# winddori2002/DEX-TTS

Hardware: AMD Instinct MI355X
Metric: mel-frames/s at n_timesteps=50, 80-ch mel (sampler only); RTF (higher is better)
Workload: dtype bf16; 1 GPU; gedex_b1: gedex_lj B=1/GPU T=512 n_timesteps=50 (BASELINE.json configs[1]); global_batch=1, frames=512, hipgraph=False, parallelism=1 GPU

## Files before the change

### dex_tts_amd/csrc/conv_down.hip

```cpp
#include "kernels.h"
#include <cstdlib>
#include "lp_util.h"
#include "kernels_lp.h"

namespace dex {
namespace DEX_LP_NS {

typedef float f32x16 __attribute__((ext_vector_type(16)));
typedef unsigned short u16;

namespace {
constexpr int CD_C = 64, CD_MPX = 64, CD_PXB = 144;
constexpr int CD_PL = CD_MPX + 1, CD_ROWB = 2 * CD_PL * CD_PXB;
constexpr int CD_NIT = (2 * CD_MPX + 1) * 8, CD_NL = (CD_NIT + 255) / 256;
}

template <bool ALP> struct CdRow;
template <> struct CdRow<true> { uint4 a[CD_NL]; float m[CD_NL]; };
template <> struct CdRow<false> { uint4 a[CD_NL]; uint4 c[CD_NL]; float m[CD_NL]; };

template <bool ALP, bool CLP>
#ifdef DEX_LP_WSPLIT
#define CD_WAVES_ATTR
#else
#define CD_WAVES_ATTR __attribute__((amdgpu_waves_per_eu(ALP ? 2 : 1, ALP ? 2 : 1)))
#endif
__global__ __launch_bounds__(256) CD_WAVES_ATTR void conv_down_kernel(const ConvDownP p) {
    constexpr int SPB = CLP ? 144 : 272, STG = CD_MPX * SPB, OCH = CLP ? 8 : 16, NS = CD_MPX * OCH / 256;
    extern __shared__ __attribute__((aligned(16))) unsigned char smem_cd[];
    unsigned char* ring = smem_cd;
    unsigned char* stage = smem_cd + 3 * CD_ROWB;
    float* bs = reinterpret_cast<float*>(stage + STG);
    const int DUMMY = 3 * CD_ROWB + STG + CD_C * 4;
    const int tid = threadIdx.x, lane = tid & 63, wave = tid >> 6;
    const int i = lane & 31, hh = lane >> 5;
    const int ct = wave & 1, pt = wave >> 1;
    const int seg = blockIdx.x % p.nseg, chunk = blockIdx.x / p.nseg, b = blockIdx.y;
    const int ow0 = seg * CD_MPX, Ho = p.H / 2, Wo = p.W / 2;
    const int r0 = chunk * p.rows_per_wg, r1 = min(Ho, r0 + p.rows_per_wg);
    const bool full_strip = ow0 + CD_MPX <= Wo;
    const u16* Xb = reinterpret_cast<const u16*>(p.X) + (long)b * p.xb + p.x_coff;
    const float* Xf = reinterpret_cast<const float*>(p.X) + (long)b * p.xb + p.x_coff;
    const float* mrow = p.inmask + (long)b * p.mask_bstride;

    int coff[CD_NL], roff[CD_NL]; float cmask[CD_NL];
#pragma unroll
    for (int j = 0; j < CD_NL; ++j) {
        const int q = tid + 256 * j;
        const int pc = q >> 3, c8 = (q & 7) * 8;
        const int wi = 2 * ow0 - 1 + pc;
        const bool ok = q < CD_NIT && (unsigned)wi < (unsigned)p.W;
        const int wc = ok ? wi : 0;
        coff[j] = wc * p.ldx + c8;
        cmask[j] = ok ? mrow[wc * p.inmask_ws] : 0.f;
        roff[j] = q < CD_NIT ? ((pc & 1) * CD_PL + (pc >> 1)) * CD_PXB + c8 * 2 : -1;
    }
    using Row = CdRow<ALP>;
    auto row_load = [&](int row, Row& R) __attribute__((always_inline)) {
        const bool rok = (unsigned)row < (unsigned)p.H;
        const int rc = __builtin_amdgcn_readfirstlane(rok ? row : 0);
#pragma unroll
        for (int j = 0; j < CD_NL; ++j) {
            if constexpr (ALP) R.a[j] = *reinterpret_cast<const uint4*>(Xb + (long)rc * p.W * p.ldx + coff[j]);
            else { const float* xf = Xf + (long)rc * p.W * p.ldx + coff[j]; R.a[j] = *reinterpret_cast<const uint4*>(xf); R.c[j] = *reinterpret_cast<const uint4*>(xf + 4); }
            R.m[j] = rok ? cmask[j] : 0.f;
        }
    };
    auto row_store = [&](int row, const Row& R) __attribute__((always_inline)) {
        const int slot = __builtin_amdgcn_readfirstlane((row + 1) % 3) * CD_ROWB;
#pragma unroll
        for (int j = 0; j < CD_NL; ++j) {
            const float m = R.m[j];
            uint4 v;
            if constexpr (ALP) {
                v.x = pack2_lp(lp_lo(R.a[j].x) * m, lp_hi(R.a[j].x) * m); v.y = pack2_lp(lp_lo(R.a[j].y) * m, lp_hi(R.a[j].y) * m);
                v.z = pack2_lp(lp_lo(R.a[j].z) * m, lp_hi(R.a[j].z) * m); v.w = pack2_lp(lp_lo(R.a[j].w) * m, lp_hi(R.a[j].w) * m);
            } else {
                v.x = pack2_lp(__uint_as_float(R.a[j].x) * m, __uint_as_float(R.a[j].y) * m); v.y = pack2_lp(__uint_as_float(R.a[j].z) * m, __uint_as_float(R.a[j].w) * m);
                v.z = pack2_lp(__uint_as_float(R.c[j].x) * m, __uint_as_float(R.c[j].y) * m); v.w = pack2_lp(__uint_as_float(R.c[j].z) * m, __uint_as_float(R.c[j].w) * m);
            }
            *reinterpret_cast<uint4*>(smem_cd + (roff[j] >= 0 ? slot + roff[j] : DUMMY)) = v;
        }
    };

    Row Ra, Rb;
    row_load(2 * r0 - 1, Ra);
    row_load(2 * r0, Rb);
    uint4 wr[36];
    {
        const uint4* Wf = reinterpret_cast<const uint4*>(p.Wfrag) + (long)ct * 36 * 64 + lane;
#pragma unroll
        for (int ks = 0; ks < 36; ++ks) wr[ks] = Wf[ks * 64];
    }
#ifdef DEX_LP_WSPLIT
    uint4 wl[36];
    {
        const uint4* Wf = reinterpret_cast<const uint4*>(p.Wfrag) + 2L * 36 * 64 + (long)ct * 36 * 64 + lane;
#pragma unroll
        for (int ks = 0; ks < 36; ++ks) wl[ks] = Wf[ks * 64];
    }
#endif
    if (tid < CD_C) bs[tid] = p.bias[tid];
    row_store(2 * r0 - 1, Ra);
    row_store(2 * r0, Rb);
    row_load(2 * r0 + 1, Ra);
    row_store(2 * r0 + 1, Ra);
    row_load(r0 + 1 < r1 ? 2 * r0 + 2 : -1, Ra);
    row_load(r0 + 1 < r1 ? 2 * r0 + 3 : -1, Rb);
    lds_barrier();

    for (int oh = r0; oh < r1; ++oh) {
        f32x16 acc;
#pragma unroll
        for (int r = 0; r < 16; ++r) acc[r] = 0.f;
#pragma unroll
        for (int kh = 0; kh < 3; ++kh) {
            const unsigned char* rowp = ring + __builtin_amdgcn_readfirstlane((2 * oh + kh) % 3) * CD_ROWB;
#pragma unroll
            for (int kw = 0; kw < 3; ++kw) {
                const unsigned char* xr = rowp + ((kw & 1) * CD_PL + pt * 32 + i + (kw >> 1)) * CD_PXB + hh * 16;
#pragma unroll
                for (int ks = 0; ks < 4; ++ks) {
                    const lp8 xv = *reinterpret_cast<const lp8*>(xr + ks * 32);
                    acc = DEX_MFMA_LP(__builtin_bit_cast(lp8, wr[(kh * 3 + kw) * 4 + ks]), xv, acc, 0, 0, 0);
#ifdef DEX_LP_WSPLIT
                    acc = DEX_MFMA_LP(__builtin_bit_cast(lp8, wl[(kh * 3 + kw) * 4 + ks]), xv, acc, 0, 0, 0);
#endif
                }
            }
        }
        lds_barrier();
#pragma unroll
        for (int g = 0; g < 4; ++g) {
            unsigned char* d = stage + (pt * 32 + i) * SPB + (ct * 32 + 8 * g + 4 * hh) * (CLP ? 2 : 4);
            const float4 b4 = *reinterpret_cast<const float4*>(bs + ct * 32 + 8 * g + 4 * hh);
            const float v0 = acc[4 * g] + b4.x, v1 = acc[4 * g + 1] + b4.y, v2 = acc[4 * g + 2] + b4.z, v3 = acc[4 * g + 3] + b4.w;
            if constexpr (CLP) *reinterpret_cast<uint2*>(d) = make_uint2(pack2_lp(v0, v1), pack2_lp(v2, v3));
            else *reinterpret_cast<float4*>(d) = make_float4(v0, v1, v2, v3);
        }
        row_store(2 * oh + 2, Ra);
        row_store(2 * oh + 3, Rb);
        lds_barrier();
        row_load(oh + 2 < r1 ? 2 * oh + 4 : -1, Ra);
        row_load(oh + 2 < r1 ? 2 * oh + 5 : -1, Rb);
        __builtin_amdgcn_sched_barrier(0);
        {
            uint4 ov[NS];
#pragma unroll
            for (int j = 0; j < NS; ++j) { const int q = tid + 256 * j; ov[j] = *reinterpret_cast<const uint4*>(stage + (q / OCH) * SPB + (q % OCH) * 16); }
            const long rowbase = (((long)b * Ho + oh) * Wo) * p.ldy + p.y_coff;
#define CD_OUT(pred_) _Pragma("unroll") for (int j = 0; j < NS; ++j) { \
                const int q = tid + 256 * j, wo = ow0 + q / OCH, e = wo * p.ldy + (q % OCH) * (CLP ? 8 : 4); \
                if (pred_) { if constexpr (CLP) *reinterpret_cast<uint4*>(reinterpret_cast<u16*>(p.Y) + rowbase + e) = ov[j]; \
                             else *reinterpret_cast<uint4*>(reinterpret_cast<float*>(p.Y) + rowbase + e) = ov[j]; } }
            if (full_strip) { CD_OUT(true) } else { CD_OUT(wo < Wo) }
#undef CD_OUT
        }
    }
}

bool conv_down_supported(int C, int H, int W, int ldx, int ldy, int x_coff) {
#if defined(DEX_LP_WSPLIT) && !defined(DEX_WS_HAVE_DOWN)
    return false;
#endif
   
    return C == CD_C && (ldx % 8) == 0 && (ldy % 8) == 0 && (x_coff % 8) == 0 && (H % 2) == 0 && (W % 2) == 0 && H >= 2 && W >= 2;
}

void launch_conv_down(const ConvDownP& p0, hipStream_t st) {
    g_last_symbol = "conv_down_kernel";
    ConvDownP p = p0;
    const int Ho = p.H / 2, Wo = p.W / 2;
    p.nseg = (Wo + CD_MPX - 1) / CD_MPX;
    const int target = knob_or("DEX_CONV_DOWN_WGS", 512);
    int nchunk = (target + p.nseg * p.B - 1) / (p.nseg * p.B);
    if (nchunk < 1) nchunk = 1;
    if (nchunk > Ho) nchunk = Ho;
    p.rows_per_wg = (Ho + nchunk - 1) / nchunk;
    nchunk = (Ho + p.rows_per_wg - 1) / p.rows_per_wg;
    const int lds = 3 * CD_ROWB + CD_MPX * (p.c_lp ? 144 : 272) + CD_C * 4 + 16;
    static bool attr = false;
    if (!attr) {
        constexpr int LMAX = 3 * CD_ROWB + CD_MPX * 272 + CD_C * 4 + 16;
        hipFuncSetAttribute(reinterpret_cast<const void*>(&conv_down_kernel<true, true>), hipFuncAttributeMaxDynamicSharedMemorySize, LMAX);
        hipFuncSetAttribute(reinterpret_cast<const void*>(&conv_down_kernel<true, false>), hipFuncAttributeMaxDynamicSharedMemorySize, LMAX);
        hipFuncSetAttribute(reinterpret_cast<const void*>(&conv_down_kernel<false, true>), hipFuncAttributeMaxDynamicSharedMemorySize, LMAX);
        hipFuncSetAttribute(reinterpret_cast<const void*>(&conv_down_kernel<false, false>), hipFuncAttributeMaxDynamicSharedMemorySize, LMAX);
        attr = true;
    }
    const dim3 grid(p.nseg * nchunk, p.B);
    if (p.a_lp) { if (p.c_lp) hipLaunchKernelGGL((conv_down_kernel<true, true>), grid, dim3(256), lds, st, p); else hipLaunchKernelGGL((conv_down_kernel<true, false>), grid, dim3(256), lds, st, p); }
    else { if (p.c_lp) hipLaunchKernelGGL((conv_down_kernel<false, true>), grid, dim3(256), lds, st, p); else hipLaunchKernelGGL((conv_down_kernel<false, false>), grid, dim3(256), lds, st, p); }
}

}
}
```

### dex_tts_amd/csrc/convt_up.hip

```cpp
#include "kernels.h"
#include <cstdlib>
#include "lp_util.h"
#include "kernels_lp.h"

namespace dex {
namespace DEX_LP_NS {

typedef float f32x16 __attribute__((ext_vector_type(16)));
typedef unsigned short u16;

namespace {

constexpr int CU_C = 64;
constexpr int CU_PXB = 144;

template <int MT, bool ALP, bool CLP>
struct CuGeom {
    static constexpr int MPX = 32 * MT, PC = MPX + 2, ROWB = PC * CU_PXB, RING = 4 * ROWB;
    static constexpr int OPX = 2 * MPX, SPB = CLP ? 144 : 272, STG = 2 * OPX * SPB;
    static constexpr int NL = (PC * 8 + 255) / 256;
    static constexpr int OCH = CLP ? 8 : 16;
    static constexpr int NS = 2 * OPX * OCH / 256;
    static constexpr int NB = NS < 8 ? NS : 8;
    static constexpr int LDS = RING + STG + 256;
};

template <int NL, int PC, bool ALP>
__device__ __forceinline__ void cu_row_load(const ConvTUpP& p, const void* Xb, const float* mrow, int row, int iw0, int tid,
                                            uint4 (&ra)[NL], uint4 (&rb)[ALP ? 1 : NL], float (&m)[NL]) {
    const bool rok = (unsigned)row < (unsigned)p.H;
    const int rc = rok ? row : 0;
#pragma unroll
    for (int j = 0; j < NL; ++j) {
        const int q = tid + 256 * j;
        const int px = q >> 3, c8 = (q & 7) * 8;
        const int iw = iw0 - 1 + px;
        const bool ok = rok && q < PC * 8 && (unsigned)iw < (unsigned)p.W;
        const int wc = ok ? iw : 0;
        const long e = ((long)rc * p.W + wc) * p.ldx + c8;
        if constexpr (ALP) ra[j] = *reinterpret_cast<const uint4*>(reinterpret_cast<const u16*>(Xb) + e);
        else {
            ra[j] = *reinterpret_cast<const uint4*>(reinterpret_cast<const float*>(Xb) + e);
            rb[j] = *reinterpret_cast<const uint4*>(reinterpret_cast<const float*>(Xb) + e + 4);
        }
        const float mv = mrow[wc * p.inmask_ws];
        m[j] = ok ? mv : 0.f;
    }
}
template <int NL, int PC, bool ALP>
__device__ __forceinline__ void cu_row_store(unsigned char* slot, int tid, const uint4 (&ra)[NL], const uint4 (&rb)[ALP ? 1 : NL], const float (&m)[NL]) {
#pragma unroll
    for (int j = 0; j < NL; ++j) {
        const int q = tid + 256 * j;
        const int px = q >> 3, c8 = (q & 7) * 8;
        uint4 v;
        if constexpr (ALP) {
            v.x = pack2_lp(lp_lo(ra[j].x) * m[j], lp_hi(ra[j].x) * m[j]); v.y = pack2_lp(lp_lo(ra[j].y) * m[j], lp_hi(ra[j].y) * m[j]);
            v.z = pack2_lp(lp_lo(ra[j].z) * m[j], lp_hi(ra[j].z) * m[j]); v.w = pack2_lp(lp_lo(ra[j].w) * m[j], lp_hi(ra[j].w) * m[j]);
        } else {
            v.x = pack2_lp(__uint_as_float(ra[j].x) * m[j], __uint_as_float(ra[j].y) * m[j]);
            v.y = pack2_lp(__uint_as_float(ra[j].z) * m[j], __uint_as_float(ra[j].w) * m[j]);
            v.z = pack2_lp(__uint_as_float(rb[j].x) * m[j], __uint_as_float(rb[j].y) * m[j]);
            v.w = pack2_lp(__uint_as_float(rb[j].z) * m[j], __uint_as_float(rb[j].w) * m[j]);
        }
        if (q < PC * 8) *reinterpret_cast<uint4*>(slot + px * CU_PXB + c8 * 2) = v;
    }
}

}

template <int MT, bool ALP, bool CLP>
__global__ __launch_bounds__(256) void convt_up_kernel(const ConvTUpP p) {
    using G = CuGeom<MT, ALP, CLP>;
    extern __shared__ __attribute__((aligned(16))) unsigned char smem_cu[];
    unsigned char* ring = smem_cu;
    unsigned char* stage = smem_cu + G::RING;
    float* bs = reinterpret_cast<float*>(smem_cu + G::RING + G::STG);
    const int tid = threadIdx.x, lane = tid & 63, wave = tid >> 6;
    const int i = lane & 31, hh = lane >> 5;
    const int ph = wave >> 1, pw = wave & 1;
    const int seg = blockIdx.x % p.nseg, chunk = blockIdx.x / p.nseg, b = blockIdx.y;
    const int iw0 = seg * G::MPX;
    const int r0 = chunk * p.rows_per_wg, r1 = min(p.H, r0 + p.rows_per_wg);
    const void* Xb = ALP ? static_cast<const void*>(reinterpret_cast<const u16*>(p.X) + (long)b * p.xb + p.x_coff)
                         : static_cast<const void*>(reinterpret_cast<const float*>(p.X) + (long)b * p.xb + p.x_coff);
    const float* mrow = p.inmask + (long)b * p.mask_bstride;
    const int OW = 2 * p.W;

    uint4 wr[2][16];
    {
        const uint4* Wf = reinterpret_cast<const uint4*>(p.Wfrag[wave]);
#pragma unroll
        for (int ct = 0; ct < 2; ++ct)
#pragma unroll
            for (int ks = 0; ks < 16; ++ks) wr[ct][ks] = Wf[(ct * 16 + ks) * 64 + lane];
    }
#ifdef DEX_LP_WSPLIT
    uint4 wl[2][16];
    {
        const uint4* Wf = reinterpret_cast<const uint4*>(p.Wfrag[wave]) + 2L * 16 * 64;
#pragma unroll
        for (int ct = 0; ct < 2; ++ct)
#pragma unroll
            for (int ks = 0; ks < 16; ++ks) wl[ct][ks] = Wf[(ct * 16 + ks) * 64 + lane];
    }
#endif
    uint4 ra[G::NL], rb[ALP ? 1 : G::NL];
    float rm[G::NL];
    {
        uint4 pa[3][G::NL], pb[3][ALP ? 1 : G::NL];
        float pm[3][G::NL];
#pragma unroll
        for (int d = 0; d < 3; ++d) cu_row_load<G::NL, G::PC, ALP>(p, Xb, mrow, r0 + d - 1, iw0, tid, pa[d], pb[d], pm[d]);
        const float bv = tid < CU_C ? p.bias[tid] : 0.f;
        cu_row_load<G::NL, G::PC, ALP>(p, Xb, mrow, r0 + 2 <= r1 ? r0 + 2 : -1, iw0, tid, ra, rb, rm);
#pragma unroll
        for (int d = 0; d < 3; ++d) cu_row_store<G::NL, G::PC, ALP>(ring + ((r0 + d) & 3) * G::ROWB, tid, pa[d], pb[d], pm[d]);
        if (tid < CU_C) bs[tid] = bv;
    }
    lds_barrier();

    for (int ih = r0; ih < r1; ++ih) {
        f32x16 acc[2][MT];
#pragma unroll
        for (int ct = 0; ct < 2; ++ct)
#pragma unroll
            for (int g = 0; g < 4; ++g) {
                const float4 b4 = *reinterpret_cast<const float4*>(bs + ct * 32 + 8 * g + 4 * hh);
#pragma unroll
                for (int pt = 0; pt < MT; ++pt) { acc[ct][pt][4 * g] = b4.x; acc[ct][pt][4 * g + 1] = b4.y; acc[ct][pt][4 * g + 2] = b4.z; acc[ct][pt][4 * g + 3] = b4.w; }
            }
#pragma unroll
        for (int ks = 0; ks < 16; ++ks) {
            const int tap = ks >> 2, th = tap >> 1, tw = tap & 1;
            const unsigned char* xr = ring + ((ih + ph - th + 1) & 3) * G::ROWB + (i + 1 + pw - tw) * CU_PXB + ((ks & 3) * 16 + hh * 8) * 2;
#pragma unroll
            for (int pt = 0; pt < MT; ++pt) {
                const lp8 xb = *reinterpret_cast<const lp8*>(xr + pt * 32 * CU_PXB);
#pragma unroll
                for (int ct = 0; ct < 2; ++ct) {
                    acc[ct][pt] = DEX_MFMA_LP(__builtin_bit_cast(lp8, wr[ct][ks]), xb, acc[ct][pt], 0, 0, 0);
#ifdef DEX_LP_WSPLIT
                    acc[ct][pt] = DEX_MFMA_LP(__builtin_bit_cast(lp8, wl[ct][ks]), xb, acc[ct][pt], 0, 0, 0);
#endif
                }
            }
        }
        lds_barrier();
#pragma unroll
        for (int ct = 0; ct < 2; ++ct)
#pragma unroll
            for (int pt = 0; pt < MT; ++pt)
#pragma unroll
                for (int g = 0; g < 4; ++g) {
                    unsigned char* d = stage + (ph * G::OPX + 2 * (pt * 32 + i) + pw) * G::SPB + (ct * 32 + 8 * g + 4 * hh) * (CLP ? 2 : 4);
                    if constexpr (CLP) *reinterpret_cast<uint2*>(d) = make_uint2(pack2_lp(acc[ct][pt][4 * g], acc[ct][pt][4 * g + 1]), pack2_lp(acc[ct][pt][4 * g + 2], acc[ct][pt][4 * g + 3]));
                    else *reinterpret_cast<float4*>(d) = make_float4(acc[ct][pt][4 * g], acc[ct][pt][4 * g + 1], acc[ct][pt][4 * g + 2], acc[ct][pt][4 * g + 3]);
                }
        cu_row_store<G::NL, G::PC, ALP>(ring + ((ih + 3) & 3) * G::ROWB, tid, ra, rb, rm);
        lds_barrier();
        cu_row_load<G::NL, G::PC, ALP>(p, Xb, mrow, ih + 3 <= r1 ? ih + 3 : -1, iw0, tid, ra, rb, rm);
        __builtin_amdgcn_sched_barrier(0);
#pragma unroll
        for (int h0 = 0; h0 < G::NS; h0 += G::NB) {
            uint4 ov[G::NB];
#pragma unroll
            for (int j = 0; j < G::NB; ++j) {
                const int q = tid + 256 * (h0 + j);
                const int row = q / (G::OPX * G::OCH), rem = q % (G::OPX * G::OCH);
                ov[j] = *reinterpret_cast<const uint4*>(stage + (row * G::OPX + rem / G::OCH) * G::SPB + (rem % G::OCH) * 16);
            }
#pragma unroll
            for (int j = 0; j < G::NB; ++j) {
                const int q = tid + 256 * (h0 + j);
                const int row = q / (G::OPX * G::OCH), rem = q % (G::OPX * G::OCH);
                const int ow = 2 * iw0 + rem / G::OCH;
                const long e = (((long)b * 2 * p.H + 2 * ih + row) * OW + ow) * p.ldy + p.y_coff + (rem % G::OCH) * (CLP ? 8 : 4);
                if (ow < OW) {
                    if constexpr (CLP) *reinterpret_cast<uint4*>(reinterpret_cast<u16*>(p.Y) + e) = ov[j];
                    else *reinterpret_cast<uint4*>(reinterpret_cast<float*>(p.Y) + e) = ov[j];
                }
            }
        }
    }
}

bool convt_up_supported(int C, int H, int W, int ldx, int ldy) {
#if defined(DEX_LP_WSPLIT) && !defined(DEX_WS_HAVE_UP)
    return false;
#endif
    return C == CU_C && (ldx % 8) == 0 && (ldy % 8) == 0 && H >= 1 && W >= 1; }

template <int MT, bool ALP, bool CLP>
static void cu_launch(ConvTUpP p, hipStream_t st) {
    using G = CuGeom<MT, ALP, CLP>;
    static_assert(G::NS % G::NB == 0, "output chunks");
    p.nseg = (p.W + G::MPX - 1) / G::MPX;
    const long tiles = (long)p.H * p.nseg * p.B;
    const int target = knob_or("DEX_CONVT_WGS", 512);
    int R = (int)((tiles + target - 1) / target);
    if (R < 1) R = 1;
    if (R > p.H) R = p.H;
    const int nchunk = (p.H + R - 1) / R;
    p.rows_per_wg = R;
    static bool attr = false;
    if (!attr) { hipFuncSetAttribute(reinterpret_cast<const void*>(&convt_up_kernel<MT, ALP, CLP>), hipFuncAttributeMaxDynamicSharedMemorySize, G::LDS); attr = true; }
    hipLaunchKernelGGL((convt_up_kernel<MT, ALP, CLP>), dim3(p.nseg * nchunk, p.B), dim3(256), G::LDS, st, p);
}

void launch_convt_up(const ConvTUpP& p, hipStream_t st) {
    g_last_symbol = "convt_up_kernel";
    const bool wide = knob_or("DEX_CONVT_MT", 0) == 2;
#define CU_GO(MT) do { if (p.a_lp && p.c_lp) cu_launch<MT, true, true>(p, st); else if (p.a_lp) cu_launch<MT, true, false>(p, st); \
                       else if (p.c_lp) cu_launch<MT, false, true>(p, st); else cu_launch<MT, false, false>(p, st); } while (0)
    if (wide) CU_GO(2); else CU_GO(1);
#undef CU_GO
}

}
}
```

### dex_tts_amd/csrc/dex_api.hip

```cpp
#include <hip/hip_runtime.h>
#include <cstdlib>

#include <cmath>
#include <cstdarg>
#include <atomic>
#include <cstdio>
#include <mutex>
#include <cstring>
#include <map>
#include <unordered_map>
#include <string_view>
#include <string>
#include <vector>

#include "../../include/dex_amd.h"
#include "kernels.h"
#include "weight_store.h"

using namespace dex;

namespace dex {
namespace {
const char* const KNOB_NAMES[] = {
    "DEX_CONV_STREAM", "DEX_CONV_PP", "DEX_CONV_SKIP_DEAD", "DEX_H_BF16", "DEX_ATTN_SEPARATE", "DEX_ATTN_Q64", "DEX_ATTN_Q64_TAIL", "DEX_ATTN_Q64_HALF", "DEX_DIT_XCDS", "DEX_ATTN_GENERIC", "DEX_RES2", "DEX_LP_INTER", "DEX_DIT_CHAIN",
    "DEX_DIT_CLUSTER", "DEX_DIT_CLUSTER_LOCAL", "DEX_ATTN_X_LP", "DEX_RES_X_LP", "DEX_CAT_LP", "DEX_XCD_MAP", "DEX_DEBUG_DROP_HANDOFF", "DEX_PATCH_FUSED",
    "DEX_CONV_DOWN", "DEX_CONVT_UP", "DEX_DEBUG_PLAN",
    "DEX_ATTN_SHARED_W8", "DEX_CONVT_MT", "DEX_CONVT_WGS", "DEX_CONV_DOWN_WGS", "DEX_CONV_REGW", "DEX_CONV_REGW_RES", "DEX_CONV_SMALL_MAX", "DEX_CONV_TH8",
    "DEX_CONV_W8", "DEX_DWCONV_CAP", "DEX_FINAL_CAP", "DEX_FIRST_CAP", "DEX_FIRST_MFMA", "DEX_GEMM_NWALK", "DEX_NWALK_SPLIT", "DEX_NWALK_BM", "DEX_POS_COL", "DEX_POS_COL_MIN",
    "DEX_POS_CT", "DEX_REGW_MIN_TILES", "DEX_REGW_WGS", "DEX_ROWCHAIN64", "DEX_ROWCHAIN64A", "DEX_TIV_CAP", "DEX_TV_CHAIN", "DEX_TIV_FOLD", "DEX_LINATTN_NSUB", "DEX_TV_FOLD", "DEX_OUT2_MIN", "DEX_NWALK_DMA",
    "DEX_LINATTN_HEADWAVES", "DEX_LINATTN_OUT2_HW", "DEX_CONV_ROUND1", "DEX_CONV_RESIDENT", "DEX_KVCTX_ROWS", "DEX_OUT2_ROWS", "DEX_PE_TOK", "DEX_NWALK_SMALL"};
constexpr int N_KNOBS = (int)(sizeof(KNOB_NAMES) / sizeof(KNOB_NAMES[0]));
int knob_parse(const char* e) {
    if (!e) return KNOB_UNSET;
    char* end = nullptr;
    const long v = strtol(e, &end, 10);
    if (end == e) {
        static bool warned = false;
        if (!warned) { warned = true; fprintf(stderr, "libdexamd: ignoring a DEX_* knob whose value '%s' is not an integer\n", e); }
        return KNOB_UNSET;
    }
    return (int)v;
}
struct KnobSnapshot {
    int v[N_KNOBS];
    KnobSnapshot() { for (int i = 0; i < N_KNOBS; ++i) v[i] = knob_parse(getenv(KNOB_NAMES[i])); }
};
thread_local const KnobSnapshot* t_knobs = nullptr;
struct WsplitScope {
    bool prev;
    explicit WsplitScope(bool on) : prev(g_lp_wsplit) { g_lp_wsplit = on; }
    ~WsplitScope() { g_lp_wsplit = prev; }
};
struct KnobScope {
    const KnobSnapshot* prev;
    explicit KnobScope(const KnobSnapshot* k) : prev(t_knobs) { t_knobs = k; }
    ~KnobScope() { t_knobs = prev; }
};
}
static int knob_index(const char* name) {
    static const std::unordered_map<std::string_view, int> idx = [] {
        std::unordered_map<std::string_view, int> m;
        for (int i = 0; i < N_KNOBS; ++i) m.emplace(KNOB_NAMES[i], i);
        return m;
    }();
    const auto it = idx.find(std::string_view(name));
    return it == idx.end() ? -1 : it->second;
}
int knob(const char* name) {
    if (t_knobs) {
        const int i = knob_index(name);
        if (i >= 0) return t_knobs->v[i];
    }
    return knob_parse(getenv(name));
}
}
static_assert(PREC_FP32 == DEX_PREC_FP32 && PREC_BF16 == DEX_PREC_BF16 && PREC_FP16 == DEX_PREC_FP16 && PREC_FP16X2 == DEX_PREC_FP16X2, "kernels.h mirrors DexPrecision");

namespace {
void xcd_map_probe();

struct TD { float* p; int ld; int coff; int C; int lp = 0; };

struct ResW { PackedW w1, w2, wr; const float *b1, *g1, *be1, *b2, *g2, *be2, *br, *mlp_w, *mlp_b; int cin, cout; };
constexpr int ATT_KSPLIT_MAX = 4;
static int att_split_cap(long tokens) { return tokens <= 20480 ? 8 : ATT_KSPLIT_MAX; }
static bool attention_q64_regime(int N, int B) {
    if (N < 1024) return dit_sep64_small_n(N, B) && dit_rowchain64_form(N, B, 0);
    const int ks = attention_q64_ksplit(N, B, att_split_cap((long)B * N));
    const int nt32 = (N + 31) / 32, ng = (nt32 + 7) / 8;
    return 2L * B * ng * ks >= 128;
}
struct LinW { PackedW wqkv; const float *wqkv_raw, *wout_raw, *bias_eff, *g; LpView wkv[3], wq_frag[3]; int C; };
struct DitBlockW { PackedW wqkv, wproj, wfc1, wfc2; const float *bqkv, *bproj, *bfc1, *bfc2, *ada_w, *ada_b; };

struct Prof { std::string name; hipEvent_t a, b; double flops, bytes; };
struct ProfAgg { std::string name; int calls; double ms, flops, bytes; };

struct Arena {
    char* base = nullptr; size_t off = 0, cap = 0; bool dry = true;
    void* take(size_t bytes) {
        off = (off + 255) & ~size_t(255);
        void* p = dry ? nullptr : (void*)(base + off);
        if (!dry && trace) fprintf(stderr, "plan[%d] off %zu bytes %zu\n", trace++, off, bytes);
        off += bytes;
        return p;
    }
    int trace = 0;
    float* f(size_t n) { return (float*)take(n * sizeof(float)); }
};

}

struct DexCtx : WeightStore {
    DexCtx() : WeightStore("") {}
    DexConfig cfg{};
    int lpi() const { return precision == DEX_PREC_FP16X2 ? 2 : precision == DEX_PREC_FP16 ? 1 : 0; }
    int lp_kind() const { return precision == DEX_PREC_BF16 ? 1 : 2; }
    bool lp() const { return precision != DEX_PREC_FP32; }
    bool tuned = true;
    int precision = DEX_PREC_FP32;
    std::vector<std::vector<ResW>> down_res, up_res;
    std::vector<LinW> down_lin, up_lin;
    std::vector<PackedW> down_ds_w;
    std::vector<std::vector<PackedW>> up_us_w;
    std::vector<const float*> down_ds_b, up_us_b;
    const float *fc_w3 = nullptr, *fc_w1 = nullptr;
    PackedW fin_w, pe_pw, fl_w, tv_wk, tv_wv, tv_wl;
    PackedW pos_w;
    const float *fin_b = nullptr, *fin_g = nullptr, *fin_be = nullptr, *fconv_w = nullptr, *fconv_b = nullptr;
    const float *pe_dw = nullptr, *pe_db = nullptr, *pe_pb = nullptr, *pos_b = nullptr, *freq_pos = nullptr;
    std::vector<DitBlockW> blocks;
    const float *fl_b = nullptr, *fl_ada_w = nullptr, *fl_ada_b = nullptr;
    const float *tv_wq_raw = nullptr;
    float *mel_basis = nullptr, *mel_filt = nullptr; void* mel_ws = nullptr; size_t mel_ws_bytes = 0;
    const int* last_xerr = nullptr;
    int* st_host = nullptr; hipEvent_t st_ev = nullptr; bool st_pending = false;
    struct Tap { std::string name; const float* p; std::vector<int64_t> shape; };
    std::vector<Tap> taps;
    bool prof_on = false;
    std::vector<Prof> prof;
    std::vector<ProfAgg> prof_agg;
    struct GraphEntry { std::vector<uint64_t> key; hipGraphExec_t exec; uint64_t stamp; const int* xerr; };
    std::vector<GraphEntry> graphs;
    uint64_t graph_clock = 0;
    void drop_graphs() { for (auto& g : graphs) hipGraphExecDestroy(g.exec); graphs.clear(); }
    template <typename F> int replay(const std::vector<uint64_t>& key, hipStream_t st, F&& enqueue);
    void reset_records() {
        taps.clear();
        if (prof_on) { for (auto& pr : prof) { hipEventDestroy(pr.a); hipEventDestroy(pr.b); } prof.clear(); prof_agg.clear(); }
    }
};

template <typename F> int DexCtx::replay(const std::vector<uint64_t>& key, hipStream_t st, F&& enqueue) {
    GraphEntry* hit = nullptr;
    for (auto& g : graphs) if (g.key == key) { hit = &g; break; }
    if (!hit) {
        constexpr size_t MAX_GRAPHS = 8;
        if (graphs.size() >= MAX_GRAPHS) {
            size_t lru = 0;
            for (size_t i = 1; i < graphs.size(); ++i) if (graphs[i].stamp < graphs[lru].stamp) lru = i;
            hipGraphExecDestroy(graphs[lru].exec);
            graphs.erase(graphs.begin() + lru);
        }
        hipGraph_t graph = nullptr;
        DEX_HIPCHK(this, hipStreamBeginCapture(st, hipStreamCaptureModeThreadLocal));
        const int rc = enqueue();
        hipError_t ec = hipStreamEndCapture(st, &graph);
        if (rc) { if (graph) hipGraphDestroy(graph); return rc; }
        if (ec != hipSuccess || !graph) return fail(DEX_ERR_HIP, "stream capture failed: %s", hipGetErrorString(ec));
        hipGraphExec_t exec = nullptr;
        ec = hipGraphInstantiate(&exec, graph, nullptr, nullptr, 0);
        hipGraphDestroy(graph);
        if (ec != hipSuccess) return fail(DEX_ERR_HIP, "hipGraphInstantiate failed: %s", hipGetErrorString(ec));
        graphs.push_back({key, exec, 0, last_xerr});
        hit = &graphs.back();
    }
    last_xerr = hit->xerr;
    hit->stamp = ++graph_clock;
    DEX_HIPCHK(this, hipGraphLaunch(hit->exec, st));
    DEX_HIPCHK(this, hipGetLastError());
    return DEX_OK;
}

namespace {

int stage_dim(const DexConfig& c, int i) { return c.dim * c.dim_mults[i]; }
int in_planes(const DexConfig& c) { return 2 + (c.n_spks > 1 ? 1 : 0); }
int mid_dim(const DexConfig& c) { return stage_dim(c, c.n_stages - 1); }
int mid_h(const DexConfig& c) { return c.n_feats >> (c.n_stages - 1); }
int grid_h(const DexConfig& c) { return mid_h(c) / c.dit_stride; }
int token_rows(const DexConfig& c) { return (mid_h(c) + 2 * (c.dit_patch / 2) - c.dit_patch) / c.dit_stride + 1; }
int token_cols(const DexConfig& c, int wmid) {
    const int p = c.dit_patch, s = c.dit_stride;
    const int wp = (wmid % p == 0) ? wmid : wmid + (p - wmid % p);
    return (wp + 2 * (p / 2) - p) / s + 1;
}
int mlp_hidden(const DexConfig& c) { return (int)(c.dit_hidden * c.dit_mlp_ratio); }

void add_resnet(DexCtx* x, const std::string& p, int cin, int cout, int tdim) {
    x->add(p + ".mlp.1.weight", {cout, tdim}); x->add(p + ".mlp.1.bias", {cout});
    for (int blk = 1; blk <= 2; ++blk) {
        const std::string q = p + ".block" + std::to_string(blk) + ".block";
        x->add(q + ".0.weight", {cout, blk == 1 ? cin : cout, 3, 3}); x->add(q + ".0.bias", {cout});
        x->add(q + ".1.weight", {cout}); x->add(q + ".1.bias", {cout});
    }
    if (cin != cout) { x->add(p + ".res_conv.weight", {cout, cin, 1, 1}); x->add(p + ".res_conv.bias", {cout}); }
}
void add_linattn(DexCtx* x, const std::string& p, int c) {
    x->add(p + ".fn.g", {1});
    x->add(p + ".fn.fn.to_qkv.weight", {384, c, 1, 1});
    x->add(p + ".fn.fn.to_out.weight", {c, 128, 1, 1});
    x->add(p + ".fn.fn.to_out.bias", {c});
}
void build_inventory(DexCtx* x) {
    const DexConfig& c = x->cfg;
    const int d = c.dim;
    x->add("mlp.0.weight", {4 * d, d}); x->add("mlp.0.bias", {4 * d});
    x->add("mlp.2.weight", {d, 4 * d}); x->add("mlp.2.bias", {d});
    if (c.variant == DEX_VARIANT_DEX)
        for (const char* n : {"mlp_adap", "mlp_adap_sty"}) {
            const std::string s(n);
            x->add(s + ".0.weight", {d, d}); x->add(s + ".0.bias", {d});
            x->add(s + ".2.weight", {2 * d, d}); x->add(s + ".2.bias", {2 * d});
        }
    if (c.n_spks > 1) {
        const int e = c.spk_emb_dim;
        x->add("spk_mlp.0.weight", {4 * e, e}); x->add("spk_mlp.0.bias", {4 * e});
        x->add("spk_mlp.2.weight", {c.n_feats, 4 * e}); x->add("spk_mlp.2.bias", {c.n_feats});
    }
    for (int i = 0; i < c.n_stages; ++i) {
        const int ci = i == 0 ? in_planes(c) : stage_dim(c, i - 1), co = stage_dim(c, i);
        const std::string p = "downs." + std::to_string(i);
        add_resnet(x, p + ".0", ci, co, d); add_resnet(x, p + ".1", co, co, d); add_linattn(x, p + ".2", co);
        if (i < c.n_stages - 1) { x->add(p + ".3.conv.weight", {co, co, 3, 3}); x->add(p + ".3.conv.bias", {co}); }
    }
    const int hid = c.dit_hidden, mid = mid_dim(c), mh = mlp_hidden(c);
    x->add("vit.freq_new_pos_embed", {1, hid, grid_h(c), 1});
    x->add("vit.x_embedder.proj.0.weight", {mid, 1, c.dit_patch, c.dit_patch}); x->add("vit.x_embedder.proj.0.bias", {mid});
    x->add("vit.x_embedder.proj.2.weight", {hid, mid, 1, 1}); x->add("vit.x_embedder.proj.2.bias", {hid});
    x->add("vit.t_embedder.mlp.0.weight", {hid, 256}); x->add("vit.t_embedder.mlp.0.bias", {hid});
    x->add("vit.t_embedder.mlp.2.weight", {hid, hid}); x->add("vit.t_embedder.mlp.2.bias", {hid});
    x->add("vit.pos_conv.0.weight", {hid, hid / c.dit_conv_pos_groups, c.dit_conv_pos, c.dit_conv_pos});
    x->add("vit.pos_conv.0.bias", {hid});
    for (int k = 0; k < c.dit_depth; ++k) {
        const std::string p = "vit.blocks." + std::to_string(k);
        x->add(p + ".attn.qkv.weight", {3 * hid, hid}); x->add(p + ".attn.qkv.bias", {3 * hid});
        x->add(p + ".attn.proj.weight", {hid, hid}); x->add(p + ".attn.proj.bias", {hid});
        x->add(p + ".mlp.fc1.weight", {mh, hid}); x->add(p + ".mlp.fc1.bias", {mh});
        x->add(p + ".mlp.fc2.weight", {hid, mh}); x->add(p + ".mlp.fc2.bias", {hid});
        x->add(p + ".adaLN_modulation.1.weight", {6 * hid, hid}); x->add(p + ".adaLN_modulation.1.bias", {6 * hid});
    }
    const int so = c.dit_stride * c.dit_stride * mid;
    x->add("vit.final_layer.linear.weight", {so, hid}); x->add("vit.final_layer.linear.bias", {so});
    x->add("vit.final_layer.adaLN_modulation.1.weight", {2 * hid, hid}); x->add("vit.final_layer.adaLN_modulation.1.bias", {2 * hid});
    if (c.variant == DEX_VARIANT_DEX) {
        for (const char* w : {"w_q", "w_k", "w_v", "linear"}) x->add(std::string("tv_adaptor.") + w + ".weight", {mid, mid});
        for (const char* s : {"mean_sap", "std_sap"}) {
            x->add(std::string("tiv_adaptor.") + s + ".W.weight", {1, mid});
            x->add(std::string("tiv_adaptor.") + s + ".W.bias", {1});
        }
    }
    for (int j = 0; j < c.n_stages - 1; ++j) {
        const int i = c.n_stages - 1 - j;
        const int ci = stage_dim(c, i - 1), co = stage_dim(c, i);
        const std::string p = "ups." + std::to_string(j);
        add_resnet(x, p + ".0", co * 2, ci, d); add_resnet(x, p + ".1", ci, ci, d); add_linattn(x, p + ".2", ci);
        x->add(p + ".3.conv.weight", {ci, ci, 4, 4}); x->add(p + ".3.conv.bias", {ci});
    }
    x->add("final_block.block.0.weight", {d, d, 3, 3}); x->add("final_block.block.0.bias", {d});
    x->add("final_block.block.1.weight", {d}); x->add("final_block.block.1.bias", {d});
    x->add("final_conv.weight", {1, d, 1, 1}); x->add("final_conv.bias", {1});
}

__global__ void pack_convt_kernel(const float* src, float* dst, int Cin, int Cout) {
    const long total = 4L * 4 * Cin * Cout;
    for (long i = (long)blockIdx.x * blockDim.x + threadIdx.x; i < total; i += (long)gridDim.x * blockDim.x) {
        const int co = (int)(i % Cout);
        const int ci = (int)((i / Cout) % Cin);
        const int tap = (int)((i / ((long)Cout * Cin)) % 4);
        const int par = (int)(i / ((long)Cout * Cin * 4));
        const int ph = par >> 1, pw = par & 1, th = tap >> 1, tw = tap & 1;
        const int kh = (ph ? 0 : 1) + 2 * th, kw = (pw ? 0 : 1) + 2 * tw;
        dst[i] = src[(((long)ci * Cout + co) * 4 + kh) * 4 + kw];
    }
}

}

extern "C" {

const char* dex_version(void) { return "dexamd 0.1 (gfx950)"; }

int dex_ctx_create(const DexConfig* cfg, DexCtx** out) {
    if (!cfg || !out) return DEX_ERR_ARG;
    DexCtx* x = new DexCtx();
    x->cfg = *cfg;
    const DexConfig& c = x->cfg;
    *out = x;
    if (c.n_feats != 80) return x->fail(DEX_ERR_ARG, "n_feats must be 80 (diffusion.py:226 hard-codes it)");
    if (c.n_stages < 2 || c.n_stages > 4) return x->fail(DEX_ERR_ARG, "n_stages must be in [2,4]");
    if (c.dim != 64 && c.dim != 128) return x->fail(DEX_ERR_ARG, "dim must be 64 (GeDEX, DEX-VCTK/ESD) or 128 (DEX-LibriTTS)");
    if (c.dit_heads < 1 || c.dit_hidden % c.dit_heads || !attention_head_dim_supported(c.dit_hidden / c.dit_heads))
        return x->fail(DEX_ERR_ARG, "DiT head_dim must be 64, 128, 192 or 256 (hidden %d heads %d)", c.dit_hidden, c.dit_heads);
    if (c.dit_hidden % 64 || c.dit_hidden > 512) return x->fail(DEX_ERR_ARG, "dit_hidden must be a multiple of 64, <= 512");
    if (mlp_hidden(c) % 64) return x->fail(DEX_ERR_ARG, "mlp hidden must be a multiple of 64");
    if (c.dit_conv_pos_groups < 1 || c.dit_hidden % c.dit_conv_pos_groups || (c.dit_hidden / c.dit_conv_pos_groups) % 16 ||
        c.dit_hidden / c.dit_conv_pos_groups > 64)
        return x->fail(DEX_ERR_ARG, "pos-conv groups must be 16, 32, 48 or 64 channels wide");
    if (c.dit_conv_pos % 2) return x->fail(DEX_ERR_ARG, "conv_pos must be even");
    if (c.variant == DEX_VARIANT_DEX && !attention_head_dim_supported(mid_dim(c)))
        return x->fail(DEX_ERR_ARG, "DEX adaptors need mid_dim 64, 128, 192 or 256 (the cross-attention's head_dim)");
    x->tuned = c.dim == 64 && c.dit_hidden == 256 && c.dit_heads == 2 && c.dit_hidden / c.dit_conv_pos_groups == 32 &&
               (c.variant != DEX_VARIANT_DEX || mid_dim(c) == 128);
    build_inventory(x);
    xcd_map_probe();
    return DEX_OK;
}

void dex_ctx_destroy(DexCtx* x) {
    if (!x) return;
    x->release();
    if (x->mel_basis) hipFree(x->mel_basis);
    if (x->mel_filt) hipFree(x->mel_filt);
    if (x->mel_ws) hipFree(x->mel_ws);
    x->drop_graphs();
    for (auto& pr : x->prof) { hipEventDestroy(pr.a); hipEventDestroy(pr.b); }
    if (x->st_ev) hipEventDestroy(x->st_ev);
    if (x->st_host) hipHostFree(x->st_host);
    delete x;
}

const char* dex_last_error(const DexCtx* x) { return x ? x->err.c_str() : "null context"; }
int dex_ctx_num_weights(const DexCtx* x) { return x ? (int)x->keys.size() : 0; }
// ... 1608 lines not shown
```

### dex_tts_amd/csrc/dit_elem.hip

```cpp
#include "kernels.h"
#include <cstdlib>

namespace dex {

__device__ __forceinline__ float silu_d(float x) { return x * __builtin_amdgcn_rcpf(1.f + __expf(-x)); }
__device__ __forceinline__ float gelu_d(float x) { return 0.5f * x * (1.0f + erff(x * 0.70710678118654752440f)); }

template <int KS>
__global__ __launch_bounds__(256) void dwconv_silu_kernel(const DwConvP p) {
    extern __shared__ __attribute__((aligned(16))) float4 wsh_dw[];
    const int C4 = p.C >> 2;
    for (int q = threadIdx.x; q < KS * KS * C4; q += 256) wsh_dw[q] = *reinterpret_cast<const float4*>(p.Wd + (long)q * 4);
    __syncthreads();
    const long total = (long)p.B * p.Hf * p.Wt * C4;
    for (long gid = (long)blockIdx.x * 256 + threadIdx.x; gid < total; gid += (long)gridDim.x * 256) {
        const int cq = (int)(gid % C4);
        const long tok = gid / C4;
        const int wt = (int)(tok % p.Wt);
        const int f = (int)((tok / p.Wt) % p.Hf);
        const int b = (int)(tok / ((long)p.Wt * p.Hf));
        const float* X = p.X + (long)b * p.xb;
        const float* mrow = p.mask ? p.mask + (long)b * p.mask_bstride : nullptr;
        float mkc[KS]; int wcl[KS];
#pragma unroll
        for (int kw = 0; kw < KS; ++kw) {
            const int wi = wt * p.s + kw - p.pad;
            const bool inw = (unsigned)wi < (unsigned)p.Wi;
            wcl[kw] = inw ? wi : 0;
            mkc[kw] = inw ? (mrow ? mrow[wcl[kw] * p.mask_ws] : 1.f) : 0.f;
        }
        float4 acc = *reinterpret_cast<const float4*>(p.bd + cq * 4);
        const float4 a4 = p.aff ? *reinterpret_cast<const float4*>(p.aff + ((long)b * 2 + 0) * p.C + cq * 4) : make_float4(1.f, 1.f, 1.f, 1.f);
        const float4 c4 = p.aff ? *reinterpret_cast<const float4*>(p.aff + ((long)b * 2 + 1) * p.C + cq * 4) : make_float4(0.f, 0.f, 0.f, 0.f);
#pragma unroll
        for (int kh = 0; kh < KS; ++kh) {
            const int hi = f * p.s + kh - p.pad;
            const bool inh = (unsigned)hi < (unsigned)p.Hi;
            const int hc = inh ? hi : 0;
#pragma unroll
            for (int kw = 0; kw < KS; ++kw) {
                float4 v = *reinterpret_cast<const float4*>(X + ((long)hc * p.Wi + wcl[kw]) * p.ldx + cq * 4);
                if (p.aff) { v.x = fmaf(v.x, a4.x, c4.x); v.y = fmaf(v.y, a4.y, c4.y); v.z = fmaf(v.z, a4.z, c4.z); v.w = fmaf(v.w, a4.w, c4.w); }
                const float4 w = wsh_dw[(kh * KS + kw) * C4 + cq];
                const float mk = inh ? mkc[kw] : 0.f;
                acc.x = fmaf(v.x * mk, w.x, acc.x); acc.y = fmaf(v.y * mk, w.y, acc.y);
                acc.z = fmaf(v.z * mk, w.z, acc.z); acc.w = fmaf(v.w * mk, w.w, acc.w);
            }
        }
        acc.x = silu_d(acc.x); acc.y = silu_d(acc.y); acc.z = silu_d(acc.z); acc.w = silu_d(acc.w);
        *reinterpret_cast<float4*>(p.Y + tok * p.C + cq * 4) = acc;
    }
}
template <int KS>
__global__ __launch_bounds__(256) void dwconv_silu_direct_kernel(const DwConvP p) {
    const int C4 = p.C >> 2;
    const long total = (long)p.B * p.Hf * p.Wt * C4;
    const long gid = (long)blockIdx.x * 256 + threadIdx.x;
    if (gid >= total) return;
    const int cq = (int)(gid % C4);
    const long tok = gid / C4;
    const int wt = (int)(tok % p.Wt);
    const int f = (int)((tok / p.Wt) % p.Hf);
    const int b = (int)(tok / ((long)p.Wt * p.Hf));
    const float* X = p.X + (long)b * p.xb;
    const float* mrow = p.mask ? p.mask + (long)b * p.mask_bstride : nullptr;
    float4 acc = *reinterpret_cast<const float4*>(p.bd + cq * 4);
    const float4 a4 = p.aff ? *reinterpret_cast<const float4*>(p.aff + ((long)b * 2 + 0) * p.C + cq * 4) : make_float4(1.f, 1.f, 1.f, 1.f);
    const float4 c4 = p.aff ? *reinterpret_cast<const float4*>(p.aff + ((long)b * 2 + 1) * p.C + cq * 4) : make_float4(0.f, 0.f, 0.f, 0.f);
#pragma unroll
    for (int kh = 0; kh < KS; ++kh) {
        const int hi = f * p.s + kh - p.pad;
#pragma unroll
        for (int kw = 0; kw < KS; ++kw) {
            const int wi = wt * p.s + kw - p.pad;
            const bool inb = (unsigned)hi < (unsigned)p.Hi && (unsigned)wi < (unsigned)p.Wi;
            const int hc = inb ? hi : 0, wc = inb ? wi : 0;
            float4 v = *reinterpret_cast<const float4*>(X + ((long)hc * p.Wi + wc) * p.ldx + cq * 4);
            if (p.aff) { v.x = fmaf(v.x, a4.x, c4.x); v.y = fmaf(v.y, a4.y, c4.y); v.z = fmaf(v.z, a4.z, c4.z); v.w = fmaf(v.w, a4.w, c4.w); }
            const float4 w = *reinterpret_cast<const float4*>(p.Wd + (kh * KS + kw) * p.C + cq * 4);
            float mk = mrow ? mrow[wc * p.mask_ws] : 1.f;
            mk = inb ? mk : 0.f;
            acc.x = fmaf(v.x * mk, w.x, acc.x); acc.y = fmaf(v.y * mk, w.y, acc.y);
            acc.z = fmaf(v.z * mk, w.z, acc.z); acc.w = fmaf(v.w * mk, w.w, acc.w);
        }
    }
    acc.x = silu_d(acc.x); acc.y = silu_d(acc.y); acc.z = silu_d(acc.z); acc.w = silu_d(acc.w);
    *reinterpret_cast<float4*>(p.Y + tok * p.C + cq * 4) = acc;
}
void launch_dwconv_silu(const DwConvP& p, hipStream_t st) {
    const long total = (long)p.B * p.Hf * p.Wt * (p.C / 4);
    long blocks = (total + 255) / 256;
    if (blocks < 1024 || p.k < 7) {
        const dim3 g1((unsigned)blocks);
        if (p.k == 7) hipLaunchKernelGGL(dwconv_silu_direct_kernel<7>, g1, dim3(256), 0, st, p);
        else if (p.k == 3) hipLaunchKernelGGL(dwconv_silu_direct_kernel<3>, g1, dim3(256), 0, st, p);
        else if (p.k == 15) hipLaunchKernelGGL(dwconv_silu_direct_kernel<15>, g1, dim3(256), 0, st, p);
        return;
    }
    const long cap = knob_or("DEX_DWCONV_CAP", 1024);
    if (blocks > cap) blocks = cap;
    const dim3 grid((unsigned)blocks);
    const size_t lds = (size_t)p.k * p.k * p.C * sizeof(float);
    static size_t attr_bytes = 0;
    if (lds > attr_bytes) {
        hipFuncSetAttribute(reinterpret_cast<const void*>(&dwconv_silu_kernel<3>), hipFuncAttributeMaxDynamicSharedMemorySize, (int)lds);
        hipFuncSetAttribute(reinterpret_cast<const void*>(&dwconv_silu_kernel<7>), hipFuncAttributeMaxDynamicSharedMemorySize, (int)lds);
        hipFuncSetAttribute(reinterpret_cast<const void*>(&dwconv_silu_kernel<15>), hipFuncAttributeMaxDynamicSharedMemorySize, (int)lds);
        attr_bytes = lds;
    }
    if (p.k == 7) hipLaunchKernelGGL(dwconv_silu_kernel<7>, grid, dim3(256), lds, st, p);
    else if (p.k == 3) hipLaunchKernelGGL(dwconv_silu_kernel<3>, grid, dim3(256), lds, st, p);
    else if (p.k == 15) hipLaunchKernelGGL(dwconv_silu_kernel<15>, grid, dim3(256), lds, st, p);
}

__global__ __launch_bounds__(256) void pos_finish_kernel(const PosFinishP p) {
    __shared__ float4 red[4][64];
    const int tid = threadIdx.x, wt = blockIdx.x, b = blockIdx.y;
    const int D4 = p.D >> 2;
    for (int c0 = 0; c0 < D4; c0 += 64) {
        const int cq = c0 + (tid & 63), fl = tid >> 6;
        const bool act = cq < D4;
        float4 part = make_float4(0.f, 0.f, 0.f, 0.f);
        if (act) {
            const float4 bias = *reinterpret_cast<const float4*>(p.bias + cq * 4);
            const int c = cq * 4;
            const int pcol = p.cg ? (c / p.cg) * p.cg_pad + c % p.cg : c;
            const long pld = p.cg ? (long)(p.D / p.cg) * p.cg_pad : p.D;
            for (int f = fl; f < p.Hf; f += 4) {
                const long row = ((long)b * p.Hf + f) * p.Wt + wt;
                float4 a = bias;
#pragma unroll 8
                for (int s = 0; s < p.nsplit; ++s) {
                    const float4 v = *reinterpret_cast<const float4*>(p.part + (long)s * p.split_stride + row * pld + pcol);
                    a.x += v.x; a.y += v.y; a.z += v.z; a.w += v.w;
                }
                part.x += gelu_d(a.x); part.y += gelu_d(a.y); part.z += gelu_d(a.z); part.w += gelu_d(a.w);
            }
        }
        __syncthreads();
        red[fl][tid & 63] = part;
        __syncthreads();
        if (act) {
            const float inv = 1.f / (float)p.Hf;
            float4 pos;
            pos.x = (red[0][tid & 63].x + red[1][tid & 63].x + red[2][tid & 63].x + red[3][tid & 63].x) * inv;
            pos.y = (red[0][tid & 63].y + red[1][tid & 63].y + red[2][tid & 63].y + red[3][tid & 63].y) * inv;
            pos.z = (red[0][tid & 63].z + red[1][tid & 63].z + red[2][tid & 63].z + red[3][tid & 63].z) * inv;
            pos.w = (red[0][tid & 63].w + red[1][tid & 63].w + red[2][tid & 63].w + red[3][tid & 63].w) * inv;
            for (int f = fl; f < p.Hf; f += 4) {
                const long row = ((long)b * p.Hf + f) * p.Wt + wt;
                const float4 e = *reinterpret_cast<const float4*>(p.emb + row * p.D + cq * 4);
                const float4 fp = *reinterpret_cast<const float4*>(p.freq_pos + (long)f * p.D + cq * 4);
                float4 o;
                o.x = e.x + pos.x + fp.x; o.y = e.y + pos.y + fp.y; o.z = e.z + pos.z + fp.z; o.w = e.w + pos.w + fp.w;
                *reinterpret_cast<float4*>(p.tok + row * p.D + cq * 4) = o;
            }
        }
    }
}
void launch_pos_finish(const PosFinishP& p, hipStream_t st) {
    hipLaunchKernelGGL(pos_finish_kernel, dim3(p.Wt, p.B), dim3(256), 0, st, p);
}

__global__ __launch_bounds__(256) void group_pad_kernel(const float* src, float* dst, long rows, int G, int cg, int cg_pad) {
    const long total = rows * G * cg_pad;
    for (long i = (long)blockIdx.x * 256 + threadIdx.x; i < total; i += (long)gridDim.x * 256) {
        const int j = (int)(i % cg_pad);
        const long rg = i / cg_pad;
        dst[i] = j < cg ? src[rg * cg + j] : 0.f;
    }
}
void launch_group_pad(const float* src, float* dst, long rows, int G, int cg, int cg_pad, hipStream_t st) {
    long blocks = (rows * G * cg_pad + 255) / 256; if (blocks > 8192) blocks = 8192;
    hipLaunchKernelGGL(group_pad_kernel, dim3((unsigned)blocks), dim3(256), 0, st, src, dst, rows, G, cg, cg_pad);
}

__global__ __launch_bounds__(256) void ln_mod_kernel(const LnModP p) {
    const int lane = threadIdx.x & 63;
    const long row = (long)blockIdx.x * 4 + (threadIdx.x >> 6);
    const long rows = (long)p.B * p.rows_per_batch;
    if (row >= rows) return;
    const int step = p.step + (p.row_bstride ? (int)(row / p.rows_per_batch) * p.row_bstride : 0);
    const float* x = p.X + row * p.D;
    const int per = p.D >> 6;
    float v[8];
    float s = 0.f;
#pragma unroll
    for (int j = 0; j < 8; ++j) { v[j] = (j < per) ? x[lane + 64 * j] : 0.f; s += v[j]; }
    for (int o = 32; o > 0; o >>= 1) s += __shfl_xor(s, o);
    const float mean = s / (float)p.D;
    float q = 0.f;
#pragma unroll
    for (int j = 0; j < 8; ++j) { const float d = (j < per) ? v[j] - mean : 0.f; q = fmaf(d, d, q); }
    for (int o = 32; o > 0; o >>= 1) q += __shfl_xor(q, o);
    const float rstd = rsqrtf(q / (float)p.D + 1e-6f);
    const float* sh = p.shift + (long)step * p.step_stride;
    const float* sc = p.scale + (long)step * p.step_stride;
    float* y = p.Y + row * p.D;
#pragma unroll
    for (int j = 0; j < 8; ++j) {
        if (j < per) {
            const int c = lane + 64 * j;
            y[c] = (v[j] - mean) * rstd * (1.f + sc[c]) + sh[c];
        }
    }
}
void launch_ln_mod(const LnModP& p, hipStream_t st) {
    const long rows = (long)p.B * p.rows_per_batch;
    hipLaunchKernelGGL(ln_mod_kernel, dim3((unsigned)((rows + 3) / 4)), dim3(256), 0, st, p);
}

}
```

### dex_tts_amd/csrc/unet_elem.hip

```cpp
#include "kernels.h"
#include "bf16_util.h"
#include <cstdlib>

namespace dex {

__device__ __forceinline__ float mish_f(float x) {
    if (x > 20.f) return x;
    const float e = __expf(x);
    const float n = e * (e + 2.f);
    return x * (n * __builtin_amdgcn_rcpf(n + 2.f));
}
__device__ __forceinline__ float silu_f(float x) { return x * __builtin_amdgcn_rcpf(1.f + __expf(-x)); }


__device__ __forceinline__ void gn_mean_rstd(const gnfix_t* stats, int b, int groups, float* smean, float* srstd, int tid) {
    if (tid < groups * GN_SLOTS) {
        const int g = tid / GN_SLOTS;
        const longlong2 v = *reinterpret_cast<const longlong2*>(stats + (((long)b * groups + g) * GN_SLOTS + (tid % GN_SLOTS)) * 2);
        long long s1 = v.x, s2 = v.y;
        gn_slots_reduce<GN_SLOTS>(s1, s2);
        if ((tid % GN_SLOTS) == 0) gn_moments(s1, s2, 1e-5, smean[g], srstd[g]);
    }
}

template <int PLANES, int C>
__global__ __launch_bounds__(256) void first_conv_kernel(const FirstConvP p) {
    constexpr int TPP = C / 16;
    constexpr int PPB = 256 / TPP;
    constexpr int CPG = C / 8;
    __shared__ __attribute__((aligned(16))) float w3s[PLANES * 9 * C];
    __shared__ __attribute__((aligned(16))) float w1s[PLANES * C];
    __shared__ long long red[16];
    const int tid = threadIdx.x;
    for (int k = tid; k < PLANES * 9 * C; k += 256) w3s[k] = p.W3[k];
    for (int k = tid; k < PLANES * C; k += 256) w1s[k] = p.W1[k];
    if (tid < 16) red[tid] = 0;
    const int b = blockIdx.y;
    const long npu = (long)p.H * p.T;
    const int cq = tid % TPP;
    const int step = p.step + b * p.row_bstride;
    const float c_in = p.scal[step * p.scal_stride + 2];
    const float* mrow = p.mask + (long)b * p.T;
    const float* pl[2] = {p.mu + (long)b * p.H * p.T, p.x + (long)b * p.H * p.T};
    constexpr int GPT = 16 / CPG;
    float gs[GPT], gq[GPT];
#pragma unroll
    for (int g = 0; g < GPT; ++g) { gs[g] = 0.f; gq[g] = 0.f; }
    __syncthreads();
    const long ngrp = (npu + PPB - 1) / PPB;
    for (long grp = blockIdx.x; grp < ngrp; grp += gridDim.x) {
    asm volatile("" ::: "memory");
    const long pl_raw = grp * PPB + tid / TPP;
    const bool live = pl_raw < npu;
    const long pixl = live ? pl_raw : npu - 1;
    const long pix = (long)b * npu + pixl;
    const int w = (int)(pixl % p.T);
    const int h = (int)(pixl / p.T);
    float v[PLANES][9];
#pragma unroll
    for (int kh = 0; kh < 3; ++kh) {
        const int hi = h + kh - 1;
#pragma unroll
        for (int kw = 0; kw < 3; ++kw) {
            const int wi = w + kw - 1;
            const bool inb = (unsigned)hi < (unsigned)p.H && (unsigned)wi < (unsigned)p.T;
            const int hc = inb ? hi : h, wc = inb ? wi : w;
            const float mk = inb ? mrow[wc] : 0.f;
#pragma unroll
            for (int q = 0; q < PLANES; ++q) {
                float t;
                if (q < 2) t = pl[q][(long)hc * p.T + wc] * ((q == 1) ? c_in : 1.f);
                else t = p.spk[(long)b * p.H + hc];
                v[q][kh * 3 + kw] = t * mk;
            }
        }
    }
    float4 a3[4], a1[4];
#pragma unroll
    for (int j = 0; j < 4; ++j) {
        a3[j] = *reinterpret_cast<const float4*>(p.b3 + cq * 16 + j * 4);
        a1[j] = *reinterpret_cast<const float4*>(p.b1 + cq * 16 + j * 4);
    }
#pragma unroll
    for (int q = 0; q < PLANES; ++q) {
#pragma unroll
        for (int t = 0; t < 9; ++t) {
            const float x = v[q][t];
#pragma unroll
            for (int j = 0; j < 4; ++j) {
                const float4 wv = *reinterpret_cast<const float4*>(w3s + (q * 9 + t) * C + cq * 16 + j * 4);
                a3[j].x = fmaf(x, wv.x, a3[j].x); a3[j].y = fmaf(x, wv.y, a3[j].y); a3[j].z = fmaf(x, wv.z, a3[j].z); a3[j].w = fmaf(x, wv.w, a3[j].w);
            }
        }
        const float xc = v[q][4];
#pragma unroll
        for (int j = 0; j < 4; ++j) {
            const float4 w1 = *reinterpret_cast<const float4*>(w1s + q * C + cq * 16 + j * 4);
            a1[j].x = fmaf(xc, w1.x, a1[j].x); a1[j].y = fmaf(xc, w1.y, a1[j].y); a1[j].z = fmaf(xc, w1.z, a1[j].z); a1[j].w = fmaf(xc, w1.w, a1[j].w);
        }
    }
    if (live) {
        if (p.h1_bf16) {
            uint4 lo, hi;
            const int kd = p.h1_bf16;
            lo.x = pack2_kind(a3[0].x, a3[0].y, kd); lo.y = pack2_kind(a3[0].z, a3[0].w, kd); lo.z = pack2_kind(a3[1].x, a3[1].y, kd); lo.w = pack2_kind(a3[1].z, a3[1].w, kd);
            hi.x = pack2_kind(a3[2].x, a3[2].y, kd); hi.y = pack2_kind(a3[2].z, a3[2].w, kd); hi.z = pack2_kind(a3[3].x, a3[3].y, kd); hi.w = pack2_kind(a3[3].z, a3[3].w, kd);
            unsigned short* h = reinterpret_cast<unsigned short*>(p.h1) + pix * C + cq * 16;
            *reinterpret_cast<uint4*>(h) = lo;
            *reinterpret_cast<uint4*>(h + 8) = hi;
        }
#pragma unroll
        for (int j = 0; j < 4; ++j) {
            if (!p.h1_bf16) *reinterpret_cast<float4*>(p.h1 + pix * C + cq * 16 + j * 4) = a3[j];
            if (p.res) *reinterpret_cast<float4*>(p.res + pix * C + cq * 16 + j * 4) = a1[j];
        }
    }
    if (p.gn_stats) {
#pragma unroll
        for (int j = 0; j < 4; ++j) {
            const int g = (j * 4) / CPG;
            const float4 u = a3[j];
            if (live) {
                gs[g] += (u.x + u.y) + (u.z + u.w);
                gq[g] += (u.x * u.x + u.y * u.y) + (u.z * u.z + u.w * u.w);
            }
        }
    }
    }
    if (p.gn_stats) {
#pragma unroll
        for (int o = TPP; o < 64; o <<= 1) {
#pragma unroll
            for (int g = 0; g < GPT; ++g) { gs[g] += __shfl_xor(gs[g], o); gq[g] += __shfl_xor(gq[g], o); }
        }
        if ((tid & 63) < TPP) {
            const double inv_n = 1.0 / ((double)p.H * p.T * CPG);
#pragma unroll
            for (int g = 0; g < GPT; ++g) { gn_add(&red[(GPT * cq + g) * 2], gn_fix(gs[g], inv_n)); gn_add(&red[(GPT * cq + g) * 2 + 1], gn_fix(gq[g], inv_n)); }
        }
        __syncthreads();
        if (tid < 16)
            gn_add(p.gn_stats + (((long)b * 8 + (tid >> 1)) * GN_SLOTS + (blockIdx.x % GN_SLOTS)) * 2 + (tid & 1), red[tid]);
    }
}
typedef float f32x16_fc __attribute__((ext_vector_type(16)));
template <int PLANES, int C>
__global__ __launch_bounds__(256) void first_conv_mfma_kernel(const FirstConvP p) {
    constexpr int NT = C / 32, CPG = C / 8, KS = PLANES == 3 ? 2 : 1;
    __shared__ long long red[16];
    const int tid = threadIdx.x, lane = tid & 63, wave = tid >> 6;
    const int i = lane & 31, hh = lane >> 5;
    const int b = blockIdx.y;
    const long npu = (long)p.H * p.T;
    const int step = p.step + b * p.row_bstride;
    const float c_in = p.scal[step * p.scal_stride + 2];
    const float* mrow = p.mask + (long)b * p.T;
    const float* plane = (hh == 0 ? p.mu : p.x) + (long)b * npu;
    const float psc = hh == 0 ? 1.f : c_in;
    if (tid < 16) red[tid] = 0;
    float w3[KS][9][NT], w1[KS][NT], b3[NT], b1[NT];
#pragma unroll
    for (int nt = 0; nt < NT; ++nt) {
        b3[nt] = p.b3[nt * 32 + i]; b1[nt] = p.b1[nt * 32 + i];
#pragma unroll
        for (int ks = 0; ks < KS; ++ks) {
            const int pln = ks * 2 + hh;
            const bool has = pln < PLANES;
            w1[ks][nt] = has ? p.W1[pln * C + nt * 32 + i] : 0.f;
#pragma unroll
            for (int t = 0; t < 9; ++t) w3[ks][t][nt] = has ? p.W3[(pln * 9 + t) * C + nt * 32 + i] : 0.f;
        }
    }
    float gs[NT], gq[NT];
#pragma unroll
    for (int nt = 0; nt < NT; ++nt) { gs[nt] = 0.f; gq[nt] = 0.f; }
    __syncthreads();
    const long nseg = (npu + 31) / 32;
    auto gather = [&](long seg, float (&a)[KS][9]) __attribute__((always_inline)) {
        const long pl_raw = seg * 32 + i;
        const long pixl = pl_raw < npu ? pl_raw : npu - 1;
        const int w = (int)(pixl % p.T), h = (int)(pixl / p.T);
#pragma unroll
        for (int kh = 0; kh < 3; ++kh) {
            const int hi = h + kh - 1;
#pragma unroll
            for (int kw = 0; kw < 3; ++kw) {
                const int wi = w + kw - 1;
                const bool inb = (unsigned)hi < (unsigned)p.H && (unsigned)wi < (unsigned)p.T;
                const int hc = inb ? hi : h, wc = inb ? wi : w;
                const float mk = inb ? mrow[wc] : 0.f;
                const float t0 = plane[(long)hc * p.T + wc] * psc;
                a[0][kh * 3 + kw] = t0 * mk;
                if constexpr (PLANES == 3) a[1][kh * 3 + kw] = hh == 0 ? p.spk[(long)b * p.H + hc] * mk : 0.f;
            }
        }
    };
    const long nwaves = (long)gridDim.x * 4, wv = (long)blockIdx.x * 4 + wave;
    const int nstrip = p.T / 32;
    const bool strip = (p.T % 32) == 0 && nwaves >= nstrip;
    const int cs = strip ? (int)(wv % nstrip) : 0;
    float mkc[3] = {0.f, 0.f, 0.f};
    if (strip) {
#pragma unroll
        for (int kw = 0; kw < 3; ++kw) { const int wi = cs * 32 + i + kw - 1; mkc[kw] = (unsigned)wi < (unsigned)p.T ? mrow[wi] : 0.f; }
    }
    auto gather_row = [&](int hi, float (&a)[KS][9], int slot) __attribute__((always_inline)) {
        const bool rin = (unsigned)hi < (unsigned)p.H;
        const int hc = rin ? hi : 0;
        const float sp = (PLANES == 3 && hh == 0) ? p.spk[(long)b * p.H + hc] : 0.f;
#pragma unroll
        for (int kw = 0; kw < 3; ++kw) {
            const int wi = cs * 32 + i + kw - 1;
            const int wc = (unsigned)wi < (unsigned)p.T ? wi : cs * 32 + i;
            const float mk = rin ? mkc[kw] : 0.f;
            a[0][slot * 3 + kw] = (plane[(long)hc * p.T + wc] * psc) * mk;
            if constexpr (PLANES == 3) a[1][slot * 3 + kw] = sp * mk;
        }
    };
    long seg, seg_end, sstride;
    if (strip) {
        const int nrc = (int)(nwaves / nstrip), rc = (int)(wv / nstrip);
        const int R = (p.H + nrc - 1) / nrc, h0 = rc * R, h1 = rc < nrc ? min(p.H, h0 + R) : h0;
        seg = (long)h0 * nstrip + cs; seg_end = (long)h1 * nstrip; sstride = nstrip;
    } else { seg = wv; seg_end = nseg; sstride = nwaves; }
    float a[KS][9], an[KS][9];
    if (seg < seg_end) {
        if (strip) { const int h = (int)(seg / nstrip); gather_row(h - 1, a, 0); gather_row(h, a, 1); gather_row(h + 1, a, 2); }
        else gather(seg, a);
    }
    for (; seg < seg_end; seg += sstride) {
        if (seg + sstride < seg_end) {
            if (strip) {
#pragma unroll
                for (int ks = 0; ks < KS; ++ks)
#pragma unroll
                    for (int t = 0; t < 6; ++t) an[ks][t] = a[ks][t + 3];
                gather_row((int)(seg / nstrip) + 2, an, 2);
            } else gather(seg + sstride, an);
        }
        f32x16_fc acc[NT], accr[NT];
#pragma unroll
        for (int nt = 0; nt < NT; ++nt)
#pragma unroll
            for (int r = 0; r < 16; ++r) { acc[nt][r] = 0.f; accr[nt][r] = 0.f; }
#pragma unroll
        for (int t = 0; t < 9; ++t)
#pragma unroll
            for (int ks = 0; ks < KS; ++ks)
#pragma unroll
                for (int nt = 0; nt < NT; ++nt) acc[nt] = __builtin_amdgcn_mfma_f32_32x32x2f32(a[ks][t], w3[ks][t][nt], acc[nt], 0, 0, 0);
        if (p.res) {
#pragma unroll
            for (int ks = 0; ks < KS; ++ks)
#pragma unroll
                for (int nt = 0; nt < NT; ++nt) accr[nt] = __builtin_amdgcn_mfma_f32_32x32x2f32(a[ks][4], w1[ks][nt], accr[nt], 0, 0, 0);
        }
        const long p0 = seg * 32 + 4 * hh;
        const bool full = seg * 32 + 32 <= npu;
        const bool odd = (lane & 1) != 0;
#pragma unroll
        for (int nt = 0; nt < NT; ++nt) {
            const int n = nt * 32 + i;
            float v[16];
#pragma unroll
            for (int r = 0; r < 16; ++r) {
                v[r] = acc[nt][r] + b3[nt];
                const bool ok = full || p0 + (r & 3) + 8 * (r >> 2) < npu;
                const float vs = ok ? v[r] : 0.f;
                gs[nt] += vs; gq[nt] = fmaf(vs, vs, gq[nt]);
            }
            if (p.h1_bf16 && full) {
                unsigned short* hp = reinterpret_cast<unsigned short*>(p.h1) + ((long)b * npu + p0) * C + n + (odd ? 16 * C - 1 : 0);
#pragma unroll
                for (int j = 0; j < 8; ++j) {
                    const float lo_r = v[j], hi_r = v[8 + j];
                    const float recv = lane_xor1(odd ? lo_r : hi_r);
                    const float mine = odd ? hi_r : lo_r;
                    const unsigned pk = odd ? pack2_kind(recv, mine, p.h1_bf16) : pack2_kind(mine, recv, p.h1_bf16);
                    *reinterpret_cast<unsigned*>(hp + ((j & 3) + 8 * (j >> 2)) * C) = pk;
                }
            } else {
#pragma unroll
                for (int r = 0; r < 16; ++r) {
                    const long pr = p0 + (r & 3) + 8 * (r >> 2);
                    if (pr < npu) {
                        if (p.h1_bf16) reinterpret_cast<unsigned short*>(p.h1)[((long)b * npu + pr) * C + n] = (unsigned short)(pack2_kind(v[r], 0.f, p.h1_bf16) & 0xffffu);
                        else p.h1[((long)b * npu + pr) * C + n] = v[r];
                    }
                }
            }
            if (p.res) {
#pragma unroll
                for (int r = 0; r < 16; ++r) {
                    const long pr = p0 + (r & 3) + 8 * (r >> 2);
                    if (pr < npu) p.res[((long)b * npu + pr) * C + n] = accr[nt][r] + b1[nt];
                }
            }
        }
#pragma unroll
        for (int ks = 0; ks < KS; ++ks)
#pragma unroll
            for (int t = 0; t < 9; ++t) a[ks][t] = an[ks][t];
    }
    if (p.gn_stats) {
        const double inv_n = 1.0 / ((double)p.H * p.T * CPG);
#pragma unroll
        for (int nt = 0; nt < NT; ++nt) {
            float a_ = gs[nt], q_ = gq[nt];
            for (int o = 1; o < CPG; o <<= 1) { a_ += __shfl_xor(a_, o); q_ += __shfl_xor(q_, o); }
            a_ += __shfl_xor(a_, 32); q_ += __shfl_xor(q_, 32);
            if (hh == 0 && (i & (CPG - 1)) == 0) {
                const int g = (nt * 32 + i) / CPG;
                gn_add(&red[g * 2], gn_fix(a_, inv_n)); gn_add(&red[g * 2 + 1], gn_fix(q_, inv_n));
            }
        }
        __syncthreads();
        if (tid < 16) gn_add(p.gn_stats + (((long)b * 8 + (tid >> 1)) * GN_SLOTS + (blockIdx.x % GN_SLOTS)) * 2 + (tid & 1), red[tid]);
    }
}

void launch_first_conv(const FirstConvP& p, hipStream_t st) {
    const long npu = (long)p.H * p.T;
    const int ppb = p.C == 128 ? 32 : 64;
    long blocks = (npu + ppb - 1) / ppb;
    const long capt = knob_or("DEX_FIRST_CAP", 4096);
    const long cap = capt / p.B > 32 ? capt / p.B : 32;
    if (blocks > cap) blocks = cap;
    const int mfma = knob_or("DEX_FIRST_MFMA", 1);
    if (mfma) {
        long nb = (npu + 127) / 128;
        const long capm = knob_or("DEX_FIRST_CAP", p.B >= 8 ? 512 : 1024);
        const long cm = capm / p.B > 16 ? capm / p.B : 16;
        if (nb > cm) nb = cm;
        const dim3 g2((unsigned)nb, p.B);
        if (p.C == 128) { if (p.planes == 3) hipLaunchKernelGGL((first_conv_mfma_kernel<3, 128>), g2, dim3(256), 0, st, p); else hipLaunchKernelGGL((first_conv_mfma_kernel<2, 128>), g2, dim3(256), 0, st, p); }
        else { if (p.planes == 3) hipLaunchKernelGGL((first_conv_mfma_kernel<3, 64>), g2, dim3(256), 0, st, p); else hipLaunchKernelGGL((first_conv_mfma_kernel<2, 64>), g2, dim3(256), 0, st, p); }
        return;
    }
    const dim3 grid((unsigned)blocks, p.B);
    if (p.C == 128) {
        if (p.planes == 3) hipLaunchKernelGGL((first_conv_kernel<3, 128>), grid, dim3(256), 0, st, p);
        else hipLaunchKernelGGL((first_conv_kernel<2, 128>), grid, dim3(256), 0, st, p);
        return;
    }
    if (p.planes == 3) hipLaunchKernelGGL((first_conv_kernel<3, 64>), grid, dim3(256), 0, st, p);
    else hipLaunchKernelGGL((first_conv_kernel<2, 64>), grid, dim3(256), 0, st, p);
}

constexpr int GN_PIX = 256;
__global__ __launch_bounds__(256) void gn_stats_kernel(const GnStatsP p) {
    __shared__ long long red[32][2];
    const int tid = threadIdx.x, b = blockIdx.y;
    const int C4 = p.C >> 2, cpg = p.C / p.groups;
    if (tid < 32) { red[tid][0] = 0; red[tid][1] = 0; }
    __syncthreads();
    const int cq = tid % C4, prow = tid / C4, rpp = 256 / C4;
    const int pbeg = blockIdx.x * GN_PIX;
    const int pend = min(p.npix, pbeg + GN_PIX);
    const float* X = p.X + (long)b * p.bstride;
    float s = 0.f, ss = 0.f;
    for (int px = pbeg + prow; px < pend; px += rpp) {
        const float4 v = *reinterpret_cast<const float4*>(X + (long)px * p.ld + cq * 4);
        s += (v.x + v.y) + (v.z + v.w);
        ss += (v.x * v.x + v.y * v.y) + (v.z * v.z + v.w * v.w);
    }
    const int g = (cq * 4) / cpg;
    const double inv_n = 1.0 / ((double)p.npix * cpg);
    gn_add(&red[g][0], gn_fix(s, inv_n));
    gn_add(&red[g][1], gn_fix(ss, inv_n));
    __syncthreads();
    if (tid < p.groups * 2) {
        const int gg = tid >> 1, k = tid & 1;
        gn_add(p.stats + (((long)b * p.groups + gg) * GN_SLOTS + (blockIdx.x % GN_SLOTS)) * 2 + k, red[gg][k]);
    }
}
void launch_gn_stats(const GnStatsP& p, hipStream_t st) {
    dim3 grid((p.npix + GN_PIX - 1) / GN_PIX, p.B);
    hipLaunchKernelGGL(gn_stats_kernel, grid, dim3(256), 0, st, p);
}

__global__ __launch_bounds__(256) void gn_apply_kernel(const GnApplyP p) {
    __shared__ float smean[32], srstd[32];
    const int tid = threadIdx.x, b = blockIdx.y;
    const int C4 = p.C >> 2, cpg = p.C / p.groups;
    gn_mean_rstd(p.stats, b, p.groups, smean, srstd, tid);
    __syncthreads();
    const int step = p.step + b * p.row_bstride;
    const long total = (long)p.npix * C4;
    const float* X = p.X + (long)b * p.xb;
    float* Y = p.Y + (long)b * p.yb + p.y_coff;
    const float* R = p.res ? p.res + (long)b * p.resb : nullptr;
    const float* mrow = p.mask + (long)b * p.mask_bstride;
    for (long idx = (long)blockIdx.x * 256 + tid; idx < total; idx += (long)gridDim.x * 256) {
        const int cq = (int)(idx % C4);
        const long px = idx / C4;
        const int w = (int)(px % p.W);
        const int c = cq * 4, g = c / cpg;
        const float mean = smean[g], rstd = srstd[g];
        const float4 x = *reinterpret_cast<const float4*>(X + px * p.ldx + c);
        const float4 ga = *reinterpret_cast<const float4*>(p.gamma + c);
        const float4 be = *reinterpret_cast<const float4*>(p.beta + c);
        float4 y;
        y.x = mish_f((x.x - mean) * rstd * ga.x + be.x);
        y.y = mish_f((x.y - mean) * rstd * ga.y + be.y);
        y.z = mish_f((x.z - mean) * rstd * ga.z + be.z);
        y.w = mish_f((x.w - mean) * rstd * ga.w + be.w);
        if (p.tadd) {
            const float4 t = *reinterpret_cast<const float4*>(p.tadd + (long)step * p.tadd_step_stride + c);
            y.x += t.x; y.y += t.y; y.z += t.z; y.w += t.w;
        }
        const float mk = mrow[w * p.mask_ws];
        if (R && p.res_under_mask) {
            const float4 r = *reinterpret_cast<const float4*>(R + px * p.ldres + c);
            y.x += r.x; y.y += r.y; y.z += r.z; y.w += r.w;
        }
        y.x *= mk; y.y *= mk; y.z *= mk; y.w *= mk;
        if (R && !p.res_under_mask) {
            const float4 r = *reinterpret_cast<const float4*>(R + px * p.ldres + c);
            y.x += r.x; y.y += r.y; y.z += r.z; y.w += r.w;
        }
        *reinterpret_cast<float4*>(Y + px * p.ldy + c) = y;
    }
}
void launch_gn_apply(const GnApplyP& p, hipStream_t st) {
    const long total = (long)p.npix * (p.C / 4);
    long blocks = (total + 256 * 4 - 1) / (256 * 4);
    if (blocks > 2048) blocks = 2048;
    if (blocks < 1) blocks = 1;
    hipLaunchKernelGGL(gn_apply_kernel, dim3((unsigned)blocks, p.B), dim3(256), 0, st, p);
}

constexpr int FIN_U = 4;
template <typename PT>
__global__ __launch_bounds__(256) void final_kernel(const PT p) {
    constexpr bool GEN = std::is_same<PT, FinalGP>::value;
    constexpr bool MS = std::is_same<PT, FinalMP>::value;
    __shared__ float smean[32], srstd[32];
    const int tid = threadIdx.x, b = blockIdx.y;
    const int cpg = p.C / p.groups;
    gn_mean_rstd(p.stats, b, p.groups, smean, srstd, tid);
    __syncthreads();
    const int step = p.step + b * p.row_bstride;
    const float* sc = p.scal + (long)step * p.scal_stride;
    const float sigma = sc[0], sigma_next = sc[1], c_skip = sc[3], c_out = sc[4];
    const float* X = p.X + (long)b * p.xb;
    const unsigned short* Xh = reinterpret_cast<const unsigned short*>(p.X) + (long)b * p.xb;
    const float* mrow = p.mask + (long)b * p.mask_bstride;
    const int sub = tid & 7;
    const int nblk = p.C / 64;
    f32x2 ca[2][4], cb[2][4], cw[2][4];
#pragma unroll
    for (int k = 0; k < 2; ++k) {
        if (k < nblk) {
            const int c = k * 64 + sub * 8;
#pragma unroll
            for (int j = 0; j < 4; ++j) {
                const int c0 = c + 2 * j, c1 = c0 + 1;
                const float a0 = srstd[c0 / cpg] * p.gamma[c0], a1 = srstd[c1 / cpg] * p.gamma[c1];
                ca[k][j] = f32x2{a0, a1};
                cb[k][j] = f32x2{p.beta[c0] - smean[c0 / cpg] * a0, p.beta[c1] - smean[c1 / cpg] * a1};
                cw[k][j] = f32x2{p.wfc[c0], p.wfc[c1]};
            }
        }
    }
    const float bfc = p.bfc[0];
    const bool poisoned = p.poison && *p.poison;
    const float inv = 1.f / sigma;
    const float h = p.htab ? p.htab[step] : sigma_next - sigma;
    float gA = 0.f, gB = 0.f, gh = 0.f, gah = 0.f, gw0 = 0.f, gw1 = 0.f, gsn = 1.f;
    if constexpr (GEN) {
        const float* g = p.gtab + (long)step * 8;
        gA = g[2]; gB = g[3]; gh = g[4]; gah = g[5]; gw0 = g[6]; gw1 = g[7];
        if (p.xin_next) gsn = g[8 + 1];
    }
    float ma = 0.f, mb = 0.f, mc = 0.f;
    if constexpr (MS) {
        const float* g = p.mtab + (long)step * 8;
        ma = g[2]; mb = g[3]; mc = g[4];
    }
    const long stride = (long)gridDim.x * 32 * FIN_U;
    for (long base = (long)blockIdx.x * 32 * FIN_U; base < p.npix; base += stride) {
        uint4 raw[FIN_U][2][2];
        float mk[FIN_U], xc[FIN_U], xa[FIN_U], xd[FIN_U], xs[FIN_U], xp[FIN_U];
#pragma unroll
        for (int u = 0; u < FIN_U; ++u) {
            const long pr = base + u * 32 + (tid >> 3);
            const long px = pr < p.npix ? pr : p.npix - 1;
            const long o = (long)b * p.npix + px;
            mk[u] = mrow[(int)(px % p.W)];
            xc[u] = p.xcur[o];
            if constexpr (MS) {
                xp[u] = p.dprev_in ? p.dprev_in[o] : 0.f;
            } else {
                xa[u] = p.mode == 2 ? p.xhat[o] : 0.f;
                xd[u] = p.mode == 2 ? p.dbuf[o] : 0.f;
            }
            if constexpr (GEN) xs[u] = p.xstate[o];
#pragma unroll
            for (int k = 0; k < 2; ++k) {
                if (k < nblk) {
                    if (p.x_bf16) raw[u][k][0] = *reinterpret_cast<const uint4*>(Xh + px * p.C + k * 64 + sub * 8);
                    else {
                        raw[u][k][0] = *reinterpret_cast<const uint4*>(X + px * p.C + k * 64 + sub * 8);
                        raw[u][k][1] = *reinterpret_cast<const uint4*>(X + px * p.C + k * 64 + sub * 8 + 4);
                    }
                }
            }
        }
#pragma unroll
        for (int u = 0; u < FIN_U; ++u) {
            f32x2 acc2 = f32x2{0.f, 0.f};
#pragma unroll
            for (int k = 0; k < 2; ++k) {
                if (k < nblk) {
                    f32x2 x[4];
                    if (p.x_bf16) {
                        const uint4 r = raw[u][k][0];
                        x[0] = f32x2{lo_kind(r.x, p.x_bf16), hi_kind(r.x, p.x_bf16)}; x[1] = f32x2{lo_kind(r.y, p.x_bf16), hi_kind(r.y, p.x_bf16)};
                        x[2] = f32x2{lo_kind(r.z, p.x_bf16), hi_kind(r.z, p.x_bf16)}; x[3] = f32x2{lo_kind(r.w, p.x_bf16), hi_kind(r.w, p.x_bf16)};
                    } else {
                        const uint4 r0 = raw[u][k][0], r1 = raw[u][k][1];
                        x[0] = f32x2{__uint_as_float(r0.x), __uint_as_float(r0.y)}; x[1] = f32x2{__uint_as_float(r0.z), __uint_as_float(r0.w)};
                        x[2] = f32x2{__uint_as_float(r1.x), __uint_as_float(r1.y)}; x[3] = f32x2{__uint_as_float(r1.z), __uint_as_float(r1.w)};
                    }
#pragma unroll
                    for (int j = 0; j < 4; ++j) acc2 = mish2_add(x[j] * ca[k][j] + cb[k][j], f32x2{0.f, 0.f}) * cw[k][j] + acc2;
                }
            }
            float acc = acc2.x + acc2.y;
            acc += __shfl_xor(acc, 1); acc += __shfl_xor(acc, 2); acc += __shfl_xor(acc, 4);
            const long pr = base + u * 32 + (tid >> 3);
            if (sub == 0 && pr < p.npix) {
                const float f = (acc * mk[u] + bfc) * mk[u];
                const long o = (long)b * p.npix + pr;
                const float D = poisoned ? __builtin_nanf("") : __fadd_rn(__fmul_rn(c_skip, xc[u]), __fmul_rn(c_out, f));
                if (p.denoised) p.denoised[o] = D;
                if constexpr (MS) {
                    if (p.dprev_out) p.dprev_out[o] = D;
                    p.xnext[o] = __fadd_rn(__fadd_rn(__fmul_rn(ma, xc[u]), __fmul_rn(mb, D)), __fmul_rn(mc, xp[u]));
                } else if constexpr (GEN) {
                    const float d = __fsub_rn(__fmul_rn(gA, xs[u]), __fmul_rn(gB, D));
                    float xn;
                    if (p.mode == 2) {
                        xn = __fadd_rn(xa[u], __fmul_rn(gh, __fadd_rn(__fmul_rn(gw0, xd[u]), __fmul_rn(gw1, d))));
                    } else if (p.mode == 1) {
                        p.dbuf[o] = d;
                        xn = __fadd_rn(xs[u], __fmul_rn(gah, d));
                    } else {
                        xn = __fadd_rn(xs[u], __fmul_rn(gh, d));
                    }
                    p.xnext[o] = xn;
                    if (p.xin_next) p.xin_next[o] = __fdiv_rn(xn, gsn);
                } else if (p.xnext) {
                    const float d = __fsub_rn(__fmul_rn(inv, xc[u]), __fmul_rn(inv, D));
                    if (p.mode == 2) {
                        p.xnext[o] = __fadd_rn(xa[u], __fmul_rn(h, __fadd_rn(__fmul_rn(0.5f, xd[u]), __fmul_rn(0.5f, d))));
                    } else {
                        if (p.mode == 1) p.dbuf[o] = d;
                        p.xnext[o] = __fadd_rn(xc[u], __fmul_rn(h, d));
                    }
                }
            }
        }
    }
    if (p.zero_ptr) {
        const long nthreads = (long)gridDim.x * gridDim.y * 256;
        for (long i = ((long)blockIdx.y * gridDim.x + blockIdx.x) * 256 + tid; i < p.zero_n; i += nthreads) p.zero_ptr[i] = 0.f;
    }
}
__global__ void churn_tables_kernel(const float* sigmas, int n, float S_churn, float S_min, float S_max, float S_noise,
                                    float* t_hat, float* h, float* ncoef) {
    const int i = blockIdx.x * blockDim.x + threadIdx.x;
    if (i > n) return;
    if (i == n) { t_hat[n] = 0.f; return; }
    const float t = sigmas[i];
    const double gd = fmin((double)S_churn / (double)n, sqrt(2.0) - 1.0);
    const bool on = S_churn > 0.f && (double)S_min <= (double)t && (S_max <= 0.f || (double)t <= (double)S_max);
    const float g = on ? (float)gd : 0.f;
    const float th = __fadd_rn(t, __fmul_rn(g, t));
    t_hat[i] = th;
    h[i] = __fsub_rn(sigmas[i + 1], th);
    const float d2 = __fsub_rn(__fmul_rn(th, th), __fmul_rn(t, t));
    ncoef[i] = __fmul_rn(sqrtf(fmaxf(d2, 0.f)), S_noise);
}
void launch_churn_tables(const float* sigmas, int n, float S_churn, float S_min, float S_max, float S_noise,
                         float* t_hat, float* h, float* ncoef, hipStream_t st) {
    hipLaunchKernelGGL(churn_tables_kernel, dim3((n + 64) / 64), dim3(64), 0, st, sigmas, n, S_churn, S_min, S_max, S_noise, t_hat, h, ncoef);
}
__global__ void add_noise_kernel(float* x, const float* noise, const float* ncoef, long n) {
    const float c = *ncoef;
    for (long i = (long)blockIdx.x * blockDim.x + threadIdx.x; i < n; i += (long)gridDim.x * blockDim.x)
        x[i] = __fadd_rn(x[i], __fmul_rn(c, noise[i]));
}
void launch_add_noise(float* x, const float* noise, const float* ncoef_i, long n, hipStream_t st) {
    long blocks = (n + 255) / 256; if (blocks > 2048) blocks = 2048;
    hipLaunchKernelGGL(add_noise_kernel, dim3((unsigned)blocks), dim3(256), 0, st, x, noise, ncoef_i, n);
}
__global__ void heun_expand_kernel(const float* t_hat, const float* hin, int n, float* sig, float* h) {
    const int i = blockIdx.x * blockDim.x + threadIdx.x;
    if (i >= n) return;
    const float t = t_hat[i], hh = hin[i];
    sig[2 * i] = t; h[2 * i] = hh;
    if (i < n - 1) { sig[2 * i + 1] = t + hh; h[2 * i + 1] = hh; }
    else sig[2 * i + 1] = 0.f;
}
void launch_heun_expand(const float* t_hat, const float* hin, int n, float* sig, float* h, hipStream_t st) {
    hipLaunchKernelGGL(heun_expand_kernel, dim3((n + 63) / 64), dim3(64), 0, st, t_hat, hin, n, sig, h);
}
static long final_blocks(const FinalP& p) {
    long blocks = (p.npix + 32 * FIN_U - 1) / (32 * FIN_U);
    const long capt = knob_or("DEX_FINAL_CAP", 1536);
    const long cap = capt / p.B > 32 ? capt / p.B : 32;
    if (blocks > cap) blocks = cap;
    return blocks;
}
void launch_final(const FinalP& p, hipStream_t st) {
    hipLaunchKernelGGL(final_kernel<FinalP>, dim3((unsigned)final_blocks(p), p.B), dim3(256), 0, st, p);
}
void launch_final_general(const FinalGP& p, hipStream_t st) {
    hipLaunchKernelGGL(final_kernel<FinalGP>, dim3((unsigned)final_blocks(p), p.B), dim3(256), 0, st, p);
}
__global__ void ablation_churn_kernel(float* x, const float* noise, const float* rk, float* xin, const float* s, long n) {
    const float r = rk[0], k = rk[1];
    const float sv = xin ? *s : 1.f;
    for (long i = (long)blockIdx.x * blockDim.x + threadIdx.x; i < n; i += (long)gridDim.x * blockDim.x) {
        float v = __fmul_rn(r, x[i]);
        if (noise) v = __fadd_rn(v, __fmul_rn(k, noise[i]));
        x[i] = v;
        if (xin) xin[i] = __fdiv_rn(v, sv);
    }
}
void launch_final_multistep(const FinalMP& p, hipStream_t st) {
    hipLaunchKernelGGL(final_kernel<FinalMP>, dim3((unsigned)final_blocks(p), p.B), dim3(256), 0, st, p);
}
void launch_ablation_churn(float* x, const float* noise, const float* rk, float* xin, const float* s, long n, hipStream_t st) {
    long blocks = (n + 255) / 256; if (blocks > 2048) blocks = 2048;
    hipLaunchKernelGGL(ablation_churn_kernel, dim3((unsigned)blocks), dim3(256), 0, st, x, noise, rk, xin, s, n);
}
__global__ void ablation_init_kernel(const float* z, float* x, const float* c0, float* xin, const float* s, long n) {
    const float c = *c0;
    const float sv = xin ? *s : 1.f;
    for (long i = (long)blockIdx.x * blockDim.x + threadIdx.x; i < n; i += (long)gridDim.x * blockDim.x) {
        const float v = __fmul_rn(z[i], c);
        x[i] = v;
        if (xin) xin[i] = __fdiv_rn(v, sv);
    }
}
void launch_ablation_init(const float* z, float* x, const float* c0, float* xin, const float* s, long n, hipStream_t st) {
    long blocks = (n + 255) / 256; if (blocks > 2048) blocks = 2048;
    hipLaunchKernelGGL(ablation_init_kernel, dim3((unsigned)blocks), dim3(256), 0, st, z, x, c0, xin, s, n);
}

__global__ void cond_prep_kernel(const CondPrepP p) {
    const int i = blockIdx.x;
    const int k = threadIdx.x;
    const float sigma = p.sigmas[i], sigma_next = p.no_next ? 0.f : p.sigmas[i + 1];
    const float sd = 0.5f;
    const float c_noise = logf(sigma) / 4.f;
    if (k == 0) {
        float* sc = p.scal + (long)i * p.scal_stride;
        const float s2 = sigma * sigma + sd * sd;
        sc[0] = sigma; sc[1] = sigma_next;
        sc[2] = 1.f / sqrtf(s2);
        sc[3] = __fmul_rn(__frcp_rn(s2), sd * sd);
        sc[4] = sigma * sd / sqrtf(s2);
        sc[5] = c_noise;
    }
    const int half = p.dim / 2;
    if (k < half) {
        const float e = (float)(log(10000.0) / (double)(half - 1));
        const float f = expf((float)k * -e);
        const float a = p.pe_scale * c_noise * f;
        p.t_unet[(long)i * p.dim + k] = sinf(a);
        p.t_unet[(long)i * p.dim + half + k] = cosf(a);
    }
    if (k < 128) {
        const float f = expf((float)(-log(10000.0)) * (float)k / 128.f);
        const float a = c_noise * f;
        p.t_dit[(long)i * 256 + k] = cosf(a);
        p.t_dit[(long)i * 256 + 128 + k] = sinf(a);
    }
}
void launch_cond_prep(const CondPrepP& p, hipStream_t st) {
    hipLaunchKernelGGL(cond_prep_kernel, dim3(p.n), dim3(128), 0, st, p);
}

__global__ __launch_bounds__(256) void small_linear_kernel(const SmallLinP p) {
    const int wave = (blockIdx.x * 256 + threadIdx.x) >> 6, lane = threadIdx.x & 63;
    if (wave >= p.N) return;
    const float* w = p.W + (long)wave * p.K;
    const float bias = p.bias ? p.bias[wave] : 0.f;
    const int r0 = blockIdx.y * 8;
    float acc[8];
#pragma unroll
    for (int j = 0; j < 8; ++j) acc[j] = 0.f;
    for (int k = lane; k < p.K; k += 64) {
        const float wk = w[k];
#pragma unroll
        for (int j = 0; j < 8; ++j) {
            const int r = min(r0 + j, p.rows - 1);
            float v = p.X[(long)r * p.ldx + k];
            if (p.act_in == 1) v = mish_f(v); else if (p.act_in == 2) v = silu_f(v);
            acc[j] = fmaf(v, wk, acc[j]);
        }
    }
#pragma unroll
    for (int j = 0; j < 8; ++j) {
        float a = acc[j];
        for (int o = 32; o > 0; o >>= 1) a += __shfl_xor(a, o);
        if (lane == 0 && r0 + j < p.rows) {
            float y = a + bias;
            if (p.act_out == 1) y = mish_f(y); else if (p.act_out == 2) y = silu_f(y);
            p.Y[(long)(r0 + j) * p.ldy + wave] = y;
        }
    }
}
void launch_small_linear(const SmallLinP& p, hipStream_t st) {
    hipLaunchKernelGGL(small_linear_kernel, dim3((p.N * 64 + 255) / 256, (p.rows + 7) / 8), dim3(256), 0, st, p);
}

__global__ void scale_copy_kernel(const float* src, float* dst, long n, const float* scal) {
    const float s = scal ? *scal : 1.f;
    for (long i = (long)blockIdx.x * blockDim.x + threadIdx.x; i < n; i += (long)gridDim.x * blockDim.x) dst[i] = src[i] * s;
}
void launch_scale_copy(const float* src, float* dst, long n, const float* scal_ptr, hipStream_t st) {
    long blocks = (n + 255) / 256; if (blocks > 2048) blocks = 2048;
    hipLaunchKernelGGL(scale_copy_kernel, dim3((unsigned)blocks), dim3(256), 0, st, src, dst, n, scal_ptr);
}
__global__ void iota_kernel(int* d, int n) { const int i = blockIdx.x * blockDim.x + threadIdx.x; if (i < n) d[i] = i; }
void launch_iota(int* dst, int n, hipStream_t st) { hipLaunchKernelGGL(iota_kernel, dim3((n + 255) / 256), dim3(256), 0, st, dst, n); }
__global__ void step_reset_kernel(int* s) { *s = 0; }
__global__ void step_inc_kernel(int* s) { *s = *s + 1; }
void launch_step_reset(int* step, hipStream_t st) { hipLaunchKernelGGL(step_reset_kernel, dim3(1), dim3(1), 0, st, step); }
void launch_step_inc(int* step, hipStream_t st) { hipLaunchKernelGGL(step_inc_kernel, dim3(1), dim3(1), 0, st, step); }

__global__ void permute4_kernel(const float* src, float* dst, int d0, int d1, int d2, int d3, int p0, int p1, int p2, int p3) {
    const long n = (long)d0 * d1 * d2 * d3;
    const int sd[4] = {d0, d1, d2, d3};
    const long ss[4] = {(long)d1 * d2 * d3, (long)d2 * d3, (long)d3, 1};
    const int pm[4] = {p0, p1, p2, p3};
    for (long i = (long)blockIdx.x * blockDim.x + threadIdx.x; i < n; i += (long)gridDim.x * blockDim.x) {
        long rem = i, off = 0;
        for (int a = 3; a >= 0; --a) {
            const int dim = sd[pm[a]];
            const int idx = (int)(rem % dim);
            rem /= dim;
            off += idx * ss[pm[a]];
        }
        dst[i] = src[off];
    }
}
void launch_permute4(const float* src, float* dst, int d0, int d1, int d2, int d3, int p0, int p1, int p2, int p3, hipStream_t st) {
    const long n = (long)d0 * d1 * d2 * d3;
    long blocks = (n + 255) / 256; if (blocks > 4096) blocks = 4096; if (blocks < 1) blocks = 1;
    hipLaunchKernelGGL(permute4_kernel, dim3((unsigned)blocks), dim3(256), 0, st, src, dst, d0, d1, d2, d3, p0, p1, p2, p3);
}

__global__ void f32_to_lp_kernel(const float* src, unsigned short* dst, long n, int kind) {
    for (long i = (long)blockIdx.x * blockDim.x + threadIdx.x; i < n; i += (long)gridDim.x * blockDim.x)
        dst[i] = (unsigned short)(pack2_kind(src[i], 0.f, kind) & 0xffffu);
}
void launch_f32_to_lp(const float* src, void* dst, long n, int precision, hipStream_t st) {
    long blocks = (n + 255) / 256; if (blocks > 4096) blocks = 4096; if (blocks < 1) blocks = 1;
    hipLaunchKernelGGL(f32_to_lp_kernel, dim3((unsigned)blocks), dim3(256), 0, st, src, (unsigned short*)dst, n, precision);
}
__global__ void f32_residual_lp_kernel(const float* src, float* dst, long n, int kind) {
    for (long i = (long)blockIdx.x * blockDim.x + threadIdx.x; i < n; i += (long)gridDim.x * blockDim.x) {
        const unsigned h = pack2_kind(src[i], 0.f, kind) & 0xffffu;
        const float hf = kind == 2 ? (float)__builtin_bit_cast(_Float16, (unsigned short)h) : __uint_as_float(h << 16);
        dst[i] = src[i] - hf;
    }
}
void launch_f32_residual_lp(const float* src, float* dst, long n, int precision, hipStream_t st) {
    long blocks = (n + 255) / 256; if (blocks > 4096) blocks = 4096; if (blocks < 1) blocks = 1;
    hipLaunchKernelGGL(f32_residual_lp_kernel, dim3((unsigned)blocks), dim3(256), 0, st, src, dst, n, precision);
}
__global__ void pack_lp_nk_kernel(const float* src, unsigned short* dst, int K, int N, int kind) {
    const long total = (long)K * N;
    for (long i = (long)blockIdx.x * blockDim.x + threadIdx.x; i < total; i += (long)gridDim.x * blockDim.x) {
        const int k = (int)(i % K), n = (int)(i / K);
        dst[i] = (unsigned short)(pack2_kind(src[(long)k * N + n], 0.f, kind) & 0xffffu);
    }
}
void launch_pack_lp_nk(const float* src, void* dst, int K, int N, int precision, hipStream_t st) {
    hipLaunchKernelGGL(pack_lp_nk_kernel, dim3(256), dim3(256), 0, st, src, (unsigned short*)dst, K, N, precision);
}

void launch_spk_plane(const float* spk_out, float* plane, int B, int F, hipStream_t st) {
    launch_scale_copy(spk_out, plane, (long)B * F, nullptr, st);
}

}
```

Baseline: 29780 mel-frames/s.

## Add single-iteration kernel variants for small-batch conv, convT, final and pos-finish kernels

Adds ONE template variants of the conv_down, convt_up, first_conv, final and pos_finish kernels for launches where each workgroup handles exactly one row or tile. These variants drop the ring-buffer prefetch for the next row and the extra barriers, issue all global loads up front, and in the final kernel overlap the group-norm statistics load with the main work instead of reducing them first. They are selected by default for B=1 or small grids and can be toggled with new knobs. The change also adds timestamp instrumentation macros, and it adds template instantiations and launch-path complexity.

```diff
diff --git a/dex_tts_amd/csrc/conv_down.hip b/dex_tts_amd/csrc/conv_down.hip
--- a/dex_tts_amd/csrc/conv_down.hip
+++ b/dex_tts_amd/csrc/conv_down.hip
@@ -2,9 +2,11 @@
 #include <cstdlib>
 #include "lp_util.h"
 #include "kernels_lp.h"
+#include "step_stamps.h"
 
 namespace dex {
 namespace DEX_LP_NS {
+SE_STAMP_STATE(cd)
 
 typedef float f32x16 __attribute__((ext_vector_type(16)));
 typedef unsigned short u16;
@@ -19,7 +21,7 @@
 template <> struct CdRow<true> { uint4 a[CD_NL]; float m[CD_NL]; };
 template <> struct CdRow<false> { uint4 a[CD_NL]; uint4 c[CD_NL]; float m[CD_NL]; };
 
-template <bool ALP, bool CLP>
+template <bool ALP, bool CLP, bool ONE = false>
 #ifdef DEX_LP_WSPLIT
 #define CD_WAVES_ATTR
 #else
@@ -27,6 +29,7 @@
 #endif
 __global__ __launch_bounds__(256) CD_WAVES_ATTR void conv_down_kernel(const ConvDownP p) {
     constexpr int SPB = CLP ? 144 : 272, STG = CD_MPX * SPB, OCH = CLP ? 8 : 16, NS = CD_MPX * OCH / 256;
+    SE_DECL
     extern __shared__ __attribute__((aligned(16))) unsigned char smem_cd[];
     unsigned char* ring = smem_cd;
     unsigned char* stage = smem_cd + 3 * CD_ROWB;
@@ -37,7 +40,7 @@
     const int ct = wave & 1, pt = wave >> 1;
     const int seg = blockIdx.x % p.nseg, chunk = blockIdx.x / p.nseg, b = blockIdx.y;
     const int ow0 = seg * CD_MPX, Ho = p.H / 2, Wo = p.W / 2;
-    const int r0 = chunk * p.rows_per_wg, r1 = min(Ho, r0 + p.rows_per_wg);
+    const int r0 = chunk * p.rows_per_wg, r1 = ONE ? r0 + 1 : min(Ho, r0 + p.rows_per_wg);
     const bool full_strip = ow0 + CD_MPX <= Wo;
     const u16* Xb = reinterpret_cast<const u16*>(p.X) + (long)b * p.xb + p.x_coff;
     const float* Xf = reinterpret_cast<const float*>(p.X) + (long)b * p.xb + p.x_coff;
@@ -83,9 +86,10 @@
         }
     };
 
-    Row Ra, Rb;
+    Row Ra, Rb, Rc;
     row_load(2 * r0 - 1, Ra);
     row_load(2 * r0, Rb);
+    if constexpr (ONE) row_load(2 * r0 + 1, Rc);
     uint4 wr[36];
     {
         const uint4* Wf = reinterpret_cast<const uint4*>(p.Wfrag) + (long)ct * 36 * 64 + lane;
@@ -100,14 +104,25 @@
         for (int ks = 0; ks < 36; ++ks) wl[ks] = Wf[ks * 64];
     }
 #endif
-    if (tid < CD_C) bs[tid] = p.bias[tid];
-    row_store(2 * r0 - 1, Ra);
-    row_store(2 * r0, Rb);
-    row_load(2 * r0 + 1, Ra);
-    row_store(2 * r0 + 1, Ra);
-    row_load(r0 + 1 < r1 ? 2 * r0 + 2 : -1, Ra);
-    row_load(r0 + 1 < r1 ? 2 * r0 + 3 : -1, Rb);
+    SE_STAMP(0);
+    if constexpr (ONE) {
+        const float bv = tid < CD_C ? p.bias[tid] : 0.f;
+        __builtin_amdgcn_sched_barrier(0);
+        row_store(2 * r0 - 1, Ra);
+        row_store(2 * r0, Rb);
+        row_store(2 * r0 + 1, Rc);
+        if (tid < CD_C) bs[tid] = bv;
+    } else {
+        if (tid < CD_C) bs[tid] = p.bias[tid];
+        row_store(2 * r0 - 1, Ra);
+        row_store(2 * r0, Rb);
+        row_load(2 * r0 + 1, Ra);
+        row_store(2 * r0 + 1, Ra);
+        row_load(r0 + 1 < r1 ? 2 * r0 + 2 : -1, Ra);
+        row_load(r0 + 1 < r1 ? 2 * r0 + 3 : -1, Rb);
+    }
     lds_barrier();
+    SE_STAMP(1);
 
     for (int oh = r0; oh < r1; ++oh) {
         f32x16 acc;
@@ -129,7 +144,7 @@
                 }
             }
         }
-        lds_barrier();
+        if constexpr (!ONE) lds_barrier();
 #pragma unroll
         for (int g = 0; g < 4; ++g) {
             unsigned char* d = stage + (pt * 32 + i) * SPB + (ct * 32 + 8 * g + 4 * hh) * (CLP ? 2 : 4);
@@ -138,11 +153,16 @@
             if constexpr (CLP) *reinterpret_cast<uint2*>(d) = make_uint2(pack2_lp(v0, v1), pack2_lp(v2, v3));
             else *reinterpret_cast<float4*>(d) = make_float4(v0, v1, v2, v3);
         }
-        row_store(2 * oh + 2, Ra);
-        row_store(2 * oh + 3, Rb);
+        if constexpr (!ONE) {
+            row_store(2 * oh + 2, Ra);
+            row_store(2 * oh + 3, Rb);
+        }
         lds_barrier();
-        row_load(oh + 2 < r1 ? 2 * oh + 4 : -1, Ra);
-        row_load(oh + 2 < r1 ? 2 * oh + 5 : -1, Rb);
+        SE_STAMP(2);
+        if constexpr (!ONE) {
+            row_load(oh + 2 < r1 ? 2 * oh + 4 : -1, Ra);
+            row_load(oh + 2 < r1 ? 2 * oh + 5 : -1, Rb);
+        }
         __builtin_amdgcn_sched_barrier(0);
         {
             uint4 ov[NS];
@@ -156,7 +176,9 @@
             if (full_strip) { CD_OUT(true) } else { CD_OUT(wo < Wo) }
 #undef CD_OUT
         }
-    }
+        SE_STAMP(3);
+    }
+    SE_STORE(cd)
 }
 
 bool conv_down_supported(int C, int H, int W, int ldx, int ldy, int x_coff) {
@@ -186,9 +208,20 @@
         hipFuncSetAttribute(reinterpret_cast<const void*>(&conv_down_kernel<true, false>), hipFuncAttributeMaxDynamicSharedMemorySize, LMAX);
         hipFuncSetAttribute(reinterpret_cast<const void*>(&conv_down_kernel<false, true>), hipFuncAttributeMaxDynamicSharedMemorySize, LMAX);
         hipFuncSetAttribute(reinterpret_cast<const void*>(&conv_down_kernel<false, false>), hipFuncAttributeMaxDynamicSharedMemorySize, LMAX);
+        hipFuncSetAttribute(reinterpret_cast<const void*>(&conv_down_kernel<true, true, true>), hipFuncAttributeMaxDynamicSharedMemorySize, LMAX);
+        hipFuncSetAttribute(reinterpret_cast<const void*>(&conv_down_kernel<true, false, true>), hipFuncAttributeMaxDynamicSharedMemorySize, LMAX);
+        hipFuncSetAttribute(reinterpret_cast<const void*>(&conv_down_kernel<false, true, true>), hipFuncAttributeMaxDynamicSharedMemorySize, LMAX);
+        hipFuncSetAttribute(reinterpret_cast<const void*>(&conv_down_kernel<false, false, true>), hipFuncAttributeMaxDynamicSharedMemorySize, LMAX);
         attr = true;
     }
     const dim3 grid(p.nseg * nchunk, p.B);
+    const int one_knob = knob_or("DEX_DOWN_ONE", -1);
+    if (p.rows_per_wg == 1 && (one_knob < 0 ? p.B == 1 : one_knob != 0)) {
+        g_last_symbol = "conv_down_kernel<one>";
+        if (p.a_lp) { if (p.c_lp) hipLaunchKernelGGL((conv_down_kernel<true, true, true>), grid, dim3(256), lds, st, p); else hipLaunchKernelGGL((conv_down_kernel<true, false, true>), grid, dim3(256), lds, st, p); }
+        else { if (p.c_lp) hipLaunchKernelGGL((conv_down_kernel<false, true, true>), grid, dim3(256), lds, st, p); else hipLaunchKernelGGL((conv_down_kernel<false, false, true>), grid, dim3(256), lds, st, p); }
+        return;
+    }
     if (p.a_lp) { if (p.c_lp) hipLaunchKernelGGL((conv_down_kernel<true, true>), grid, dim3(256), lds, st, p); else hipLaunchKernelGGL((conv_down_kernel<true, false>), grid, dim3(256), lds, st, p); }
     else { if (p.c_lp) hipLaunchKernelGGL((conv_down_kernel<false, true>), grid, dim3(256), lds, st, p); else hipLaunchKernelGGL((conv_down_kernel<false, false>), grid, dim3(256), lds, st, p); }
 }
diff --git a/dex_tts_amd/csrc/convt_up.hip b/dex_tts_amd/csrc/convt_up.hip
--- a/dex_tts_amd/csrc/convt_up.hip
+++ b/dex_tts_amd/csrc/convt_up.hip
@@ -2,9 +2,11 @@
 #include <cstdlib>
 #include "lp_util.h"
 #include "kernels_lp.h"
+#include "step_stamps.h"
 
 namespace dex {
 namespace DEX_LP_NS {
+SE_STAMP_STATE(cu)
 
 typedef float f32x16 __attribute__((ext_vector_type(16)));
 typedef unsigned short u16;
@@ -69,9 +71,10 @@
 
 }
 
-template <int MT, bool ALP, bool CLP>
+template <int MT, bool ALP, bool CLP, bool ONE = false>
 __global__ __launch_bounds__(256) void convt_up_kernel(const ConvTUpP p) {
     using G = CuGeom<MT, ALP, CLP>;
+    SE_DECL
     extern __shared__ __attribute__((aligned(16))) unsigned char smem_cu[];
     unsigned char* ring = smem_cu;
     unsigned char* stage = smem_cu + G::RING;
@@ -81,7 +84,7 @@
     const int ph = wave >> 1, pw = wave & 1;
     const int seg = blockIdx.x % p.nseg, chunk = blockIdx.x / p.nseg, b = blockIdx.y;
     const int iw0 = seg * G::MPX;
-    const int r0 = chunk * p.rows_per_wg, r1 = min(p.H, r0 + p.rows_per_wg);
+    const int r0 = chunk * p.rows_per_wg, r1 = ONE ? r0 + 1 : min(p.H, r0 + p.rows_per_wg);
     const void* Xb = ALP ? static_cast<const void*>(reinterpret_cast<const u16*>(p.X) + (long)b * p.xb + p.x_coff)
                          : static_cast<const void*>(reinterpret_cast<const float*>(p.X) + (long)b * p.xb + p.x_coff);
     const float* mrow = p.inmask + (long)b * p.mask_bstride;
@@ -113,12 +116,14 @@
 #pragma unroll
         for (int d = 0; d < 3; ++d) cu_row_load<G::NL, G::PC, ALP>(p, Xb, mrow, r0 + d - 1, iw0, tid, pa[d], pb[d], pm[d]);
         const float bv = tid < CU_C ? p.bias[tid] : 0.f;
-        cu_row_load<G::NL, G::PC, ALP>(p, Xb, mrow, r0 + 2 <= r1 ? r0 + 2 : -1, iw0, tid, ra, rb, rm);
+        if constexpr (!ONE) cu_row_load<G::NL, G::PC, ALP>(p, Xb, mrow, r0 + 2 <= r1 ? r0 + 2 : -1, iw0, tid, ra, rb, rm);
+        else __builtin_amdgcn_sched_barrier(0);
 #pragma unroll
         for (int d = 0; d < 3; ++d) cu_row_store<G::NL, G::PC, ALP>(ring + ((r0 + d) & 3) * G::ROWB, tid, pa[d], pb[d], pm[d]);
         if (tid < CU_C) bs[tid] = bv;
     }
     lds_barrier();
+    SE_STAMP(0);
 
     for (int ih = r0; ih < r1; ++ih) {
         f32x16 acc[2][MT];
@@ -146,20 +151,22 @@
                 }
             }
         }
-        lds_barrier();
+        if constexpr (!ONE) lds_barrier();
 #pragma unroll
         for (int ct = 0; ct < 2; ++ct)
 #pragma unroll
             for (int pt = 0; pt < MT; ++pt)
 #pragma unroll
                 for (int g = 0; g < 4; ++g) {
+                    if (ct == 0 && pt == 0 && g == 0) SE_STAMP(1);
                     unsigned char* d = stage + (ph * G::OPX + 2 * (pt * 32 + i) + pw) * G::SPB + (ct * 32 + 8 * g + 4 * hh) * (CLP ? 2 : 4);
                     if constexpr (CLP) *reinterpret_cast<uint2*>(d) = make_uint2(pack2_lp(acc[ct][pt][4 * g], acc[ct][pt][4 * g + 1]), pack2_lp(acc[ct][pt][4 * g + 2], acc[ct][pt][4 * g + 3]));
                     else *reinterpret_cast<float4*>(d) = make_float4(acc[ct][pt][4 * g], acc[ct][pt][4 * g + 1], acc[ct][pt][4 * g + 2], acc[ct][pt][4 * g + 3]);
                 }
-        cu_row_store<G::NL, G::PC, ALP>(ring + ((ih + 3) & 3) * G::ROWB, tid, ra, rb, rm);
+        if constexpr (!ONE) cu_row_store<G::NL, G::PC, ALP>(ring + ((ih + 3) & 3) * G::ROWB, tid, ra, rb, rm);
         lds_barrier();
-        cu_row_load<G::NL, G::PC, ALP>(p, Xb, mrow, ih + 3 <= r1 ? ih + 3 : -1, iw0, tid, ra, rb, rm);
+        SE_STAMP(2);
+        if constexpr (!ONE) cu_row_load<G::NL, G::PC, ALP>(p, Xb, mrow, ih + 3 <= r1 ? ih + 3 : -1, iw0, tid, ra, rb, rm);
         __builtin_amdgcn_sched_barrier(0);
 #pragma unroll
         for (int h0 = 0; h0 < G::NS; h0 += G::NB) {
@@ -182,7 +189,9 @@
                 }
             }
         }
-    }
+        SE_STAMP(3);
+    }
+    SE_STORE(cu)
 }
 
 bool convt_up_supported(int C, int H, int W, int ldx, int ldy) {
@@ -191,6 +200,13 @@
 #endif
     return C == CU_C && (ldx % 8) == 0 && (ldy % 8) == 0 && H >= 1 && W >= 1; }
 
+template <int MT, bool ALP, bool CLP, bool ONE>
+static void cu_launch_form(const ConvTUpP& p, int nchunk, hipStream_t st) {
+    using G = CuGeom<MT, ALP, CLP>;
+    static bool attr = false;
+    if (!attr) { hipFuncSetAttribute(reinterpret_cast<const void*>(&convt_up_kernel<MT, ALP, CLP, ONE>), hipFuncAttributeMaxDynamicSharedMemorySize, G::LDS); attr = true; }
+    hipLaunchKernelGGL((convt_up_kernel<MT, ALP, CLP, ONE>), dim3(p.nseg * nchunk, p.B), dim3(256), G::LDS, st, p);
+}
 template <int MT, bool ALP, bool CLP>
 static void cu_launch(ConvTUpP p, hipStream_t st) {
     using G = CuGeom<MT, ALP, CLP>;
@@ -203,9 +219,11 @@
     if (R > p.H) R = p.H;
     const int nchunk = (p.H + R - 1) / R;
     p.rows_per_wg = R;
-    static bool attr = false;
-    if (!attr) { hipFuncSetAttribute(reinterpret_cast<const void*>(&convt_up_kernel<MT, ALP, CLP>), hipFuncAttributeMaxDynamicSharedMemorySize, G::LDS); attr = true; }
-    hipLaunchKernelGGL((convt_up_kernel<MT, ALP, CLP>), dim3(p.nseg * nchunk, p.B), dim3(256), G::LDS, st, p);
+    const int one_knob = knob_or("DEX_UP_ONE", -1);
+    if (R == 1 && (one_knob < 0 ? p.B == 1 : one_knob != 0)) {
+        g_last_symbol = "convt_up_kernel<one>";
+        cu_launch_form<MT, ALP, CLP, true>(p, nchunk, st);
+    } else cu_launch_form<MT, ALP, CLP, false>(p, nchunk, st);
 }
 
 void launch_convt_up(const ConvTUpP& p, hipStream_t st) {
diff --git a/dex_tts_amd/csrc/dex_api.hip b/dex_tts_amd/csrc/dex_api.hip
--- a/dex_tts_amd/csrc/dex_api.hip
+++ b/dex_tts_amd/csrc/dex_api.hip
@@ -28,7 +28,8 @@
     "DEX_ATTN_SHARED_W8", "DEX_CONVT_MT", "DEX_CONVT_WGS", "DEX_CONV_DOWN_WGS", "DEX_CONV_REGW", "DEX_CONV_REGW_RES", "DEX_CONV_SMALL_MAX", "DEX_CONV_TH8",
     "DEX_CONV_W8", "DEX_DWCONV_CAP", "DEX_FINAL_CAP", "DEX_FIRST_CAP", "DEX_FIRST_MFMA", "DEX_GEMM_NWALK", "DEX_NWALK_SPLIT", "DEX_NWALK_BM", "DEX_POS_COL", "DEX_POS_COL_MIN",
     "DEX_POS_CT", "DEX_REGW_MIN_TILES", "DEX_REGW_WGS", "DEX_ROWCHAIN64", "DEX_ROWCHAIN64A", "DEX_TIV_CAP", "DEX_TV_CHAIN", "DEX_TIV_FOLD", "DEX_LINATTN_NSUB", "DEX_TV_FOLD", "DEX_OUT2_MIN", "DEX_NWALK_DMA",
-    "DEX_LINATTN_HEADWAVES", "DEX_LINATTN_OUT2_HW", "DEX_CONV_ROUND1", "DEX_CONV_RESIDENT", "DEX_KVCTX_ROWS", "DEX_OUT2_ROWS", "DEX_PE_TOK", "DEX_NWALK_SMALL"};
+    "DEX_LINATTN_HEADWAVES", "DEX_LINATTN_OUT2_HW", "DEX_CONV_ROUND1", "DEX_CONV_RESIDENT", "DEX_KVCTX_ROWS", "DEX_OUT2_ROWS", "DEX_PE_TOK", "DEX_NWALK_SMALL",
+    "DEX_FINAL_ONE", "DEX_FIRST_ONE", "DEX_DOWN_ONE", "DEX_UP_ONE", "DEX_POSFIN_ONE"};
 constexpr int N_KNOBS = (int)(sizeof(KNOB_NAMES) / sizeof(KNOB_NAMES[0]));
 int knob_parse(const char* e) {
     if (!e) return KNOB_UNSET;
diff --git a/dex_tts_amd/csrc/dit_elem.hip b/dex_tts_amd/csrc/dit_elem.hip
--- a/dex_tts_amd/csrc/dit_elem.hip
+++ b/dex_tts_amd/csrc/dit_elem.hip
@@ -1,7 +1,10 @@
 #include "kernels.h"
+#include "bf16_util.h"
+#include "step_stamps.h"
 #include <cstdlib>
 
 namespace dex {
+SE_STAMP_STATE(pf)
 
 __device__ __forceinline__ float silu_d(float x) { return x * __builtin_amdgcn_rcpf(1.f + __expf(-x)); }
 __device__ __forceinline__ float gelu_d(float x) { return 0.5f * x * (1.0f + erff(x * 0.70710678118654752440f)); }
@@ -114,6 +117,7 @@
 }
 
 __global__ __launch_bounds__(256) void pos_finish_kernel(const PosFinishP p) {
+    SE_DECL
     __shared__ float4 red[4][64];
     const int tid = threadIdx.x, wt = blockIdx.x, b = blockIdx.y;
     const int D4 = p.D >> 2;
@@ -137,9 +141,11 @@
                 part.x += gelu_d(a.x); part.y += gelu_d(a.y); part.z += gelu_d(a.z); part.w += gelu_d(a.w);
             }
         }
+        SE_STAMP(0);
         __syncthreads();
         red[fl][tid & 63] = part;
         __syncthreads();
+        SE_STAMP(1);
         if (act) {
             const float inv = 1.f / (float)p.Hf;
             float4 pos;
@@ -156,9 +162,81 @@
                 *reinterpret_cast<float4*>(p.tok + row * p.D + cq * 4) = o;
             }
         }
-    }
+        SE_STAMP(2);
+    }
+    SE_STORE(pf)
+}
+constexpr int PF_ROWS = 3;
+__global__ __launch_bounds__(256) void pos_finish_one_kernel(const PosFinishP p) {
+    SE_DECL
+    __shared__ float4 red[4][64];
+    const int tid = threadIdx.x, wt = blockIdx.x, b = blockIdx.y;
+    const int D4 = p.D >> 2;
+    const int cq = tid & 63, fl = tid >> 6;
+    const bool act = cq < D4;
+    float4 part = make_float4(0.f, 0.f, 0.f, 0.f);
+    float4 v[PF_ROWS], e[PF_ROWS], fp[PF_ROWS];
+    if (act) {
+        const float4 bias = *reinterpret_cast<const float4*>(p.bias + cq * 4);
+        const int c = cq * 4;
+        const int pcol = p.cg ? (c / p.cg) * p.cg_pad + c % p.cg : c;
+        const long pld = p.cg ? (long)(p.D / p.cg) * p.cg_pad : p.D;
+#pragma unroll
+        for (int j = 0; j < PF_ROWS; ++j) {
+            const int f = fl + 4 * j;
+            if (f < p.Hf) v[j] = *reinterpret_cast<const float4*>(p.part + (((long)b * p.Hf + f) * p.Wt + wt) * pld + pcol);
+        }
+#pragma unroll
+        for (int j = 0; j < PF_ROWS; ++j) {
+            const int f = fl + 4 * j;
+            if (f < p.Hf) {
+                const long row = ((long)b * p.Hf + f) * p.Wt + wt;
+                e[j] = *reinterpret_cast<const float4*>(p.emb + row * p.D + cq * 4);
+                fp[j] = *reinterpret_cast<const float4*>(p.freq_pos + (long)f * p.D + cq * 4);
+            }
+        }
+        __builtin_amdgcn_sched_barrier(0);
+#pragma unroll
+        for (int j = 0; j < PF_ROWS; ++j) {
+            if (fl + 4 * j < p.Hf) {
+                float4 a = bias;
+                a.x += v[j].x; a.y += v[j].y; a.z += v[j].z; a.w += v[j].w;
+                part.x += gelu_d(a.x); part.y += gelu_d(a.y); part.z += gelu_d(a.z); part.w += gelu_d(a.w);
+            }
+        }
+    }
+    SE_STAMP(0);
+    red[fl][cq] = part;
+    lds_barrier();
+    SE_STAMP(1);
+    if (act) {
+        const float inv = 1.f / (float)p.Hf;
+        float4 pos;
+        pos.x = (red[0][cq].x + red[1][cq].x + red[2][cq].x + red[3][cq].x) * inv;
+        pos.y = (red[0][cq].y + red[1][cq].y + red[2][cq].y + red[3][cq].y) * inv;
+        pos.z = (red[0][cq].z + red[1][cq].z + red[2][cq].z + red[3][cq].z) * inv;
+        pos.w = (red[0][cq].w + red[1][cq].w + red[2][cq].w + red[3][cq].w) * inv;
+#pragma unroll
+        for (int j = 0; j < PF_ROWS; ++j) {
+            const int f = fl + 4 * j;
+            if (f < p.Hf) {
+                const long row = ((long)b * p.Hf + f) * p.Wt + wt;
+                float4 o;
+                o.x = e[j].x + pos.x + fp[j].x; o.y = e[j].y + pos.y + fp[j].y; o.z = e[j].z + pos.z + fp[j].z; o.w = e[j].w + pos.w + fp[j].w;
+                *reinterpret_cast<float4*>(p.tok + row * p.D + cq * 4) = o;
+            }
+        }
+    }
+    SE_STAMP(2);
+    SE_STORE(pf)
 }
 void launch_pos_finish(const PosFinishP& p, hipStream_t st) {
+    const int one_knob = knob_or("DEX_POSFIN_ONE", -1);
+    if (p.D <= 256 && p.Hf <= 4 * PF_ROWS && p.nsplit == 1 && (one_knob < 0 ? (long)p.Wt * p.B <= device_cus() : one_knob != 0)) {
+        g_last_symbol = "pos_finish_one_kernel";
+        hipLaunchKernelGGL(pos_finish_one_kernel, dim3(p.Wt, p.B), dim3(256), 0, st, p);
+        return;
+    }
     hipLaunchKernelGGL(pos_finish_kernel, dim3(p.Wt, p.B), dim3(256), 0, st, p);
 }
 
diff --git a/dex_tts_amd/csrc/step_stamps.h b/dex_tts_amd/csrc/step_stamps.h
--- /dev/null
+++ b/dex_tts_amd/csrc/step_stamps.h
@@ -0,0 +1,18 @@
+#pragma once
+#ifdef DEX_TIMING
+#define SE_STAMP_STATE(name)                                                                                              \
+    __device__ long long* name##_dbg = nullptr;                                                                           \
+    void name##_set_dbg(long long* d) { (void)hipMemcpyToSymbol(HIP_SYMBOL(name##_dbg), &d, sizeof d); }
+#define SE_DECL long long tk[8] = {0, 0, 0, 0, 0, 0, 0, 0}; const long long tk0 = __builtin_readcyclecounter(); long long tlast = tk0;
+#define SE_STAMP(k) do { const long long now_ = __builtin_readcyclecounter(); tk[k] += now_ - tlast; tlast = now_; } while (0)
+#define SE_STORE(name)                                                                                                    \
+    if (name##_dbg && threadIdx.x == 0) {                                                                                 \
+        tk[7] = __builtin_readcyclecounter() - tk0;                                                                       \
+        for (int k_ = 0; k_ < 8; ++k_) name##_dbg[((long)blockIdx.y * gridDim.x + blockIdx.x) * 8 + k_] = tk[k_];         \
+    }
+#else
+#define SE_STAMP_STATE(name)
+#define SE_DECL
+#define SE_STAMP(k) do {} while (0)
+#define SE_STORE(name)
+#endif
diff --git a/dex_tts_amd/csrc/unet_elem.hip b/dex_tts_amd/csrc/unet_elem.hip
--- a/dex_tts_amd/csrc/unet_elem.hip
+++ b/dex_tts_amd/csrc/unet_elem.hip
@@ -1,8 +1,11 @@
 #include "kernels.h"
 #include "bf16_util.h"
+#include "step_stamps.h"
 #include <cstdlib>
 
 namespace dex {
+SE_STAMP_STATE(fc)
+SE_STAMP_STATE(fk)
 
 __device__ __forceinline__ float mish_f(float x) {
     if (x > 20.f) return x;
@@ -144,9 +147,10 @@
     }
 }
 typedef float f32x16_fc __attribute__((ext_vector_type(16)));
-template <int PLANES, int C>
+template <int PLANES, int C, bool ONE = false>
 __global__ __launch_bounds__(256) void first_conv_mfma_kernel(const FirstConvP p) {
     constexpr int NT = C / 32, CPG = C / 8, KS = PLANES == 3 ? 2 : 1;
+    SE_DECL
     __shared__ long long red[16];
     const int tid = threadIdx.x, lane = tid & 63, wave = tid >> 6;
     const int i = lane & 31, hh = lane >> 5;
@@ -174,7 +178,8 @@
     float gs[NT], gq[NT];
 #pragma unroll
     for (int nt = 0; nt < NT; ++nt) { gs[nt] = 0.f; gq[nt] = 0.f; }
-    __syncthreads();
+    if constexpr (ONE) lds_barrier(); else __syncthreads();
+    SE_STAMP(0);
     const long nseg = (npu + 31) / 32;
     auto gather = [&](long seg, float (&a)[KS][9]) __attribute__((always_inline)) {
         const long pl_raw = seg * 32 + i;
@@ -229,7 +234,7 @@
         else gather(seg, a);
     }
     for (; seg < seg_end; seg += sstride) {
-        if (seg + sstride < seg_end) {
+        if (!ONE && seg + sstride < seg_end) {
             if (strip) {
 #pragma unroll
                 for (int ks = 0; ks < KS; ++ks)
@@ -249,6 +254,7 @@
             for (int ks = 0; ks < KS; ++ks)
 #pragma unroll
                 for (int nt = 0; nt < NT; ++nt) acc[nt] = __builtin_amdgcn_mfma_f32_32x32x2f32(a[ks][t], w3[ks][t][nt], acc[nt], 0, 0, 0);
+        SE_STAMP(1);
         if (p.res) {
 #pragma unroll
             for (int ks = 0; ks < KS; ++ks)
@@ -289,7 +295,16 @@
                     }
                 }
             }
-            if (p.res) {
+            if (ONE && p.res && full) {
+                float* rp = p.res + ((long)b * npu + p0) * C + n + (odd ? 16 * C - 1 : 0);
+#pragma unroll
+                for (int j = 0; j < 8; ++j) {
+                    const float lo_r = accr[nt][j] + b1[nt], hi_r = accr[nt][8 + j] + b1[nt];
+                    const float recv = lane_xor1(odd ? lo_r : hi_r);
+                    const float mine = odd ? hi_r : lo_r;
+                    *reinterpret_cast<float2*>(rp + ((j & 3) + 8 * (j >> 2)) * C) = odd ? make_float2(recv, mine) : make_float2(mine, recv);
+                }
+            } else if (p.res) {
 #pragma unroll
                 for (int r = 0; r < 16; ++r) {
                     const long pr = p0 + (r & 3) + 8 * (r >> 2);
@@ -297,6 +312,8 @@
                 }
             }
         }
+        SE_STAMP(2);
+        if constexpr (ONE) break;
 #pragma unroll
         for (int ks = 0; ks < KS; ++ks)
 #pragma unroll
@@ -314,9 +331,11 @@
                 gn_add(&red[g * 2], gn_fix(a_, inv_n)); gn_add(&red[g * 2 + 1], gn_fix(q_, inv_n));
             }
         }
-        __syncthreads();
+        if constexpr (ONE) lds_barrier(); else __syncthreads();
+        SE_STAMP(3);
         if (tid < 16) gn_add(p.gn_stats + (((long)b * 8 + (tid >> 1)) * GN_SLOTS + (blockIdx.x % GN_SLOTS)) * 2 + (tid & 1), red[tid]);
     }
+    SE_STORE(fc)
 }
 
 void launch_first_conv(const FirstConvP& p, hipStream_t st) {
@@ -333,6 +352,12 @@
         const long cm = capm / p.B > 16 ? capm / p.B : 16;
         if (nb > cm) nb = cm;
         const dim3 g2((unsigned)nb, p.B);
+        if (4 * nb >= (npu + 31) / 32 && knob_or("DEX_FIRST_ONE", 1) != 0) {
+            g_last_symbol = "first_conv_mfma_kernel<one>";
+            if (p.C == 128) { if (p.planes == 3) hipLaunchKernelGGL((first_conv_mfma_kernel<3, 128, true>), g2, dim3(256), 0, st, p); else hipLaunchKernelGGL((first_conv_mfma_kernel<2, 128, true>), g2, dim3(256), 0, st, p); }
+            else { if (p.planes == 3) hipLaunchKernelGGL((first_conv_mfma_kernel<3, 64, true>), g2, dim3(256), 0, st, p); else hipLaunchKernelGGL((first_conv_mfma_kernel<2, 64, true>), g2, dim3(256), 0, st, p); }
+            return;
+        }
         if (p.C == 128) { if (p.planes == 3) hipLaunchKernelGGL((first_conv_mfma_kernel<3, 128>), g2, dim3(256), 0, st, p); else hipLaunchKernelGGL((first_conv_mfma_kernel<2, 128>), g2, dim3(256), 0, st, p); }
         else { if (p.planes == 3) hipLaunchKernelGGL((first_conv_mfma_kernel<3, 64>), g2, dim3(256), 0, st, p); else hipLaunchKernelGGL((first_conv_mfma_kernel<2, 64>), g2, dim3(256), 0, st, p); }
         return;
@@ -431,15 +456,27 @@
 }
 
 constexpr int FIN_U = 4;
-template <typename PT>
+template <typename PT, bool ONE = false>
 __global__ __launch_bounds__(256) void final_kernel(const PT p) {
     constexpr bool GEN = std::is_same<PT, FinalGP>::value;
     constexpr bool MS = std::is_same<PT, FinalMP>::value;
+    SE_DECL
     __shared__ float smean[32], srstd[32];
     const int tid = threadIdx.x, b = blockIdx.y;
     const int cpg = p.C / p.groups;
-    gn_mean_rstd(p.stats, b, p.groups, smean, srstd, tid);
-    __syncthreads();
+    uint4 st4 = make_uint4(0u, 0u, 0u, 0u);
+    float cga = 0.f, cbe = 0.f, cwf = 0.f;
+    if constexpr (ONE) {
+        if (tid < p.groups * GN_SLOTS) {
+            const int g = tid / GN_SLOTS, k = tid % GN_SLOTS;
+            st4 = *reinterpret_cast<const uint4*>(p.stats + (((long)b * p.groups + g) * GN_SLOTS + k) * 2);
+            if (k < cpg) { const int c = g * cpg + k; cga = p.gamma[c]; cbe = p.beta[c]; cwf = p.wfc[c]; }
+        }
+    } else {
+        gn_mean_rstd(p.stats, b, p.groups, smean, srstd, tid);
+        __syncthreads();
+    }
+    SE_STAMP(0);
     const int step = p.step + b * p.row_bstride;
     const float* sc = p.scal + (long)step * p.scal_stride;
     const float sigma = sc[0], sigma_next = sc[1], c_skip = sc[3], c_out = sc[4];
@@ -451,7 +488,7 @@
     f32x2 ca[2][4], cb[2][4], cw[2][4];
 #pragma unroll
     for (int k = 0; k < 2; ++k) {
-        if (k < nblk) {
+        if (!ONE && k < nblk) {
             const int c = k * 64 + sub * 8;
 #pragma unroll
             for (int j = 0; j < 4; ++j) {
@@ -463,6 +500,7 @@
             }
         }
     }
+    SE_STAMP(1);
     const float bfc = p.bfc[0];
     const bool poisoned = p.poison && *p.poison;
     const float inv = 1.f / sigma;
@@ -507,6 +545,40 @@
                 }
             }
         }
+        if constexpr (ONE) {
+            __shared__ __attribute__((aligned(16))) float ctab[3][128];
+            __builtin_amdgcn_sched_barrier(0);
+            if (tid < p.groups * GN_SLOTS) {
+                const int g = tid / GN_SLOTS, k = tid % GN_SLOTS;
+                long long s1 = (long long)(((unsigned long long)mov_pinned(st4.y) << 32) | mov_pinned(st4.x));
+                long long s2 = (long long)(((unsigned long long)mov_pinned(st4.w) << 32) | mov_pinned(st4.z));
+                gn_slots_reduce<GN_SLOTS>(s1, s2);
+                float mean, rstd;
+                gn_moments(s1, s2, 1e-5, mean, rstd);
+                if (k < cpg) {
+                    const int c = g * cpg + k;
+                    const float a = rstd * cga;
+                    ctab[0][c] = a; ctab[1][c] = cbe - mean * a; ctab[2][c] = cwf;
+                }
+            }
+            lds_barrier();
+#pragma unroll
+            for (int k = 0; k < 2; ++k) {
+                if (k < nblk) {
+                    const int c = k * 64 + sub * 8;
+#pragma unroll
+                    for (int j = 0; j < 4; j += 2) {
+                        const float4 a4 = *reinterpret_cast<const float4*>(&ctab[0][c + 2 * j]);
+                        const float4 b4 = *reinterpret_cast<const float4*>(&ctab[1][c + 2 * j]);
+                        const float4 w4 = *reinterpret_cast<const float4*>(&ctab[2][c + 2 * j]);
+                        ca[k][j] = f32x2{a4.x, a4.y}; ca[k][j + 1] = f32x2{a4.z, a4.w};
+                        cb[k][j] = f32x2{b4.x, b4.y}; cb[k][j + 1] = f32x2{b4.z, b4.w};
+                        cw[k][j] = f32x2{w4.x, w4.y}; cw[k][j + 1] = f32x2{w4.z, w4.w};
+                    }
+                }
+            }
+        }
+        SE_STAMP(2);
 #pragma unroll
         for (int u = 0; u < FIN_U; ++u) {
             f32x2 acc2 = f32x2{0.f, 0.f};
@@ -562,11 +634,14 @@
                 }
             }
         }
+        SE_STAMP(3);
+        if constexpr (ONE) break;
     }
     if (p.zero_ptr) {
         const long nthreads = (long)gridDim.x * gridDim.y * 256;
         for (long i = ((long)blockIdx.y * gridDim.x + blockIdx.x) * 256 + tid; i < p.zero_n; i += nthreads) p.zero_ptr[i] = 0.f;
     }
+    SE_STORE(fk)
 }
 __global__ void churn_tables_kernel(const float* sigmas, int n, float S_churn, float S_min, float S_max, float S_noise,
                                     float* t_hat, float* h, float* ncoef) {
@@ -614,12 +689,20 @@
     if (blocks > cap) blocks = cap;
     return blocks;
 }
-void launch_final(const FinalP& p, hipStream_t st) {
-    hipLaunchKernelGGL(final_kernel<FinalP>, dim3((unsigned)final_blocks(p), p.B), dim3(256), 0, st, p);
-}
-void launch_final_general(const FinalGP& p, hipStream_t st) {
-    hipLaunchKernelGGL(final_kernel<FinalGP>, dim3((unsigned)final_blocks(p), p.B), dim3(256), 0, st, p);
-}
+template <typename PT>
+static void final_launch(const PT& p, hipStream_t st) {
+    const long blocks = final_blocks(p);
+    const bool one_pass = blocks * 32 * FIN_U >= p.npix && p.groups * GN_SLOTS == 256 && p.C <= 128 && p.C % (8 * p.groups) == 0;
+    const int one_knob = knob_or("DEX_FINAL_ONE", -1);
+    if (one_pass && (one_knob < 0 ? blocks * p.B <= 3L * device_cus() : one_knob != 0)) {
+        g_last_symbol = "final_one_kernel";
+        hipLaunchKernelGGL((final_kernel<PT, true>), dim3((unsigned)blocks, p.B), dim3(256), 0, st, p);
+        return;
+    }
+    hipLaunchKernelGGL((final_kernel<PT, false>), dim3((unsigned)blocks, p.B), dim3(256), 0, st, p);
+}
+void launch_final(const FinalP& p, hipStream_t st) { final_launch(p, st); }
+void launch_final_general(const FinalGP& p, hipStream_t st) { final_launch(p, st); }
 __global__ void ablation_churn_kernel(float* x, const float* noise, const float* rk, float* xin, const float* s, long n) {
     const float r = rk[0], k = rk[1];
     const float sv = xin ? *s : 1.f;
@@ -630,9 +713,7 @@
         if (xin) xin[i] = __fdiv_rn(v, sv);
     }
 }
-void launch_final_multistep(const FinalMP& p, hipStream_t st) {
-    hipLaunchKernelGGL(final_kernel<FinalMP>, dim3((unsigned)final_blocks(p), p.B), dim3(256), 0, st, p);
-}
+void launch_final_multistep(const FinalMP& p, hipStream_t st) { final_launch(p, st); }
 void launch_ablation_churn(float* x, const float* noise, const float* rk, float* xin, const float* s, long n, hipStream_t st) {
     long blocks = (n + 255) / 256; if (blocks > 2048) blocks = 2048;
     hipLaunchKernelGGL(ablation_churn_kernel, dim3((unsigned)blocks), dim3(256), 0, st, x, noise, rk, xin, s, n);
```

Measured after the change: 30080 mel-frames/s (median of 6 runs). +1.0%, better.
